# TruongKhang/cds-mvsnet

Hardware: AMD Instinct MI355X
Metric: depth-maps/sec per ref view at 640x512 N=5 D=192 (single-stage plane sweep incl. CostRegNet + regression) (higher is better)
Workload: dtype f32; 1 GPU; M1: single-stage StageNet volume 640x512, D=192, C=8, N=5 views; parallelism=single

## Files before the change

cds_mvsnet_amd/_lib.py:

```python
from __future__ import annotations

import ctypes
import os
from ctypes import c_float, c_int, c_longlong, c_void_p

_HERE = os.path.dirname(os.path.abspath(__file__))
LIB_PATH = os.environ.get("CDS_MVSNET_LIB") or os.path.join(_HERE, "libcdsmvs_hip.so")

ACT_NONE, ACT_RELU, ACT_LEAKY01, ACT_SIGMOID, ACT_TANH = 0, 1, 2, 3, 4
ACT_ACCUM = 16
AGG_ACCUMULATE, AGG_NORMALIZE, AGG_CHANNELS_LAST, AGG_FAST_POSITIONS = 1, 2, 4, 8
WARP_FAST_POSITIONS = AGG_FAST_POSITIONS
MAX_VIEWS = 8
MAX_IMAGES = 16
STAGE_STATE_WORDS = 2080
EINVAL = -1000

P = c_void_p
I = c_int
F = c_float
DB = ctypes.c_double
L = c_longlong

SIGNATURES = {
    "cds_version": [],
    "cds_chw_to_hwc_f32": [P, P, I, I, I, P],
    "cds_stage_inputs_f32": [P, P, P, P, P, P, P, P, P, P, I, I, I, I, P],
    "cds_homo_warp_f32": [P, P, P, P, I, I, I, I, I, P],
    "cds_warp_entropy_f32": [P, P, P, P, P, I, I, I, I, I, I, P],
    "cds_warp_entropy_flags_f32": [P, P, P, P, P, I, I, I, I, I, I, I, P],
    "cds_warp_aggregate_f32": [P, P, P, P, P, P, P, I, I, I, I, I, I, I, P],
    "cds_warp_entropy_window_f32": [P, P, P, P, P, I, I, I, I, I, I, I, I, P],
    "cds_warp_aggregate_window_f32": [P, P, P, P, P, P, P, I, I, I, I, I, I, I, I, P],
    "cds_warp_aggregate_bwd_f32": [P, P, P, P, P, P, P, P, P, I, I, I, I, I, I, P],
    "cds_volume_finish_f32": [P, P, P, I, I, I, I, P, P, P],
    "cds_volume_finish_bwd_f32": [P, P, P, P, P, I, I, I, I, P, P, P, P, P],
    "cds_volume_normalize_f32": [P, P, I, I, I, P],
    "cds_volume_normalize_cl_f32": [P, P, I, I, I, P],
    "cds_softargmin_conf_f32": [P, P, P, P, P, I, I, I, I, P],
    "cds_depth_hypotheses_f32": [P, P, I, I, I, I, I, I, P, P, P],
    "cds_depth_planes_f32": [P, I, I, I, P, P],
    "cds_conv3d_k3_f32": [P, P, P, P, P, I, I, I, I, I, I, I, P],
    "cds_conv3d_k3_cl_f32": [P, P, P, P, P, I, I, I, I, I, I, P],
    "cds_conv3d_sbf_f32": [P, P, P, P, P, I, I, I, I, I, I, I, P],
    "cds_conv3d_sf16_f32": [P, P, P, P, I, I, I, I, I, I, I, P, F, P, P],
    "cds_deconv3d_sbf_f32": [P, P, P, P, P, I, I, I, I, I, I, I, P],
    "cds_deconv3d_sf16_f32": [P, P, P, P, P, I, I, I, I, I, I, P, F, P, P],
    "cds_deconv3d_zm_sf16_f32": [P, P, P, P, P, I, I, I, I, I, I, P, F, P, P],
    "cds_deconv_prob_zm_f32": [P, P, P, P, P, P, I, I, I, P],
    "cds_deconv_prob_zm_sf16_f32": [P, P, P, P, P, P, I, I, I, P, F, P],
    "cds_deconv3d_zm_f32": [P, P, P, P, P, I, I, I, I, I, I, P],
    "cds_deconv3d_k3s2_f32": [P, P, P, P, P, I, I, I, I, I, I, P],
    "cds_conv2d_f32": [P, P, P, P, I, I, I, I, I, I, I, I, I, P],
    "cds_conv2d_affine_f32": [P, P, P, P, P, I, I, I, I, I, I, I, I, I, P],
    "cds_instnorm_affine_f32": [P, P, P, I, I, I, I, F, P],
    "cds_fpn_stats_parts": [I, I],
    "cds_conv2d_fpn_f32": [P, P, P, P, P, P, P, I, I, I, I, I, I, P],
    "cds_conv2d_k3_c16_f32": [P, P, P, P, P, P, I, I, I, I, P],
    "cds_dynconv_branches_sbf_f32": [P, P, P, P, P, I, I, I, I, I, P, I, P],
    "cds_dynconv_fused_sbf_f32": [P, P, P, P, P, P, P, P, F, P, P, P, I, I, I, I, I, P, I, P],
    "cds_dynconv_fused_parts": [I, I],
    "cds_conv2d_k3_relu_sbf_f32": [P, P, P, P, P, P, I, I, I, I, P],
    "cds_dynconv_blend_f32": [P, P, P, P, P, F, P, P, I, I, I, I, I, P],
    "cds_dynconv_blend_shared_f32": [P, P, P, P, P, F, P, P, I, I, I, I, I, I, P],
    "cds_blend_stats_parts": [I, I],
    "cds_dynconv_blend_stats_f32": [P, P, P, P, P, F, P, P, P, I, I, I, I, I, I, P],
    "cds_instnorm_reduce_f32": [P, I, P, P, I, I, I, I, F, P],
    "cds_instnorm_apply_f32": [P, P, P, I, I, I, I, I, I, P],
    "cds_instnorm_act_f32": [P, P, P, I, I, I, I, I, I, P],
    "cds_debug_poison_lds": [ctypes.c_uint],
    "cds_dynconv_cl_parts": [I, I],
    "cds_dynconv_cl_f32": [P, P, P, P, P, P, P, P, F, P, P, P, I, I, I, I, P, I, P],
    "cds_dynconv_cl_sf16_f32": [P, P, P, P, P, P, P, P, F, P, P, P, I, I, I, I, P, I, F, F, P],
    "cds_conv00_cl_f32": [P, P, P, P, P, P, P, F, P, P, P, I, I, I, I, P],
    "cds_conv00_cl_sf16_f32": [P, P, P, P, P, P, P, F, P, P, P, I, I, I, I, P, F, P],
    "cds_blend_cl_parts": [I, I],
    "cds_dynconv_blend_cl_f32": [P, P, P, P, P, F, P, P, P, I, I, I, I, I, I, P],
    "cds_conv2d_k3s2_cl_f32": [P, P, P, P, I, I, I, I, I, P],
    "cds_conv2d_k3s2_cl_sf16_f32": [P, P, P, P, I, I, I, I, I, F, F, P],
    "cds_fpn_cl_parts": [I, I],
    "cds_conv2d_fpn_cl_f32": [P, P, P, P, P, P, P, I, I, I, I, I, I, P],
    "cds_vis_layer1_cl_f32": [P, P, P, P, P, I, I, I, P],
    "cds_conv2d_k3_relu_cl_f32": [P, P, P, P, P, P, I, I, I, I, P],
    "cds_instnorm_stats_cl_parts": [I, I],
    "cds_instnorm_stats_cl_f32": [P, P, I, I, I, I, P],
    "cds_instnorm_apply_cl_f32": [P, P, P, P, I, I, I, I, I, I, I, P],
    "cds_curvature_stats_f32": [P, P, P, P, P, I, P],
    "cds_curvature_stats_bwd_f32": [P, P, P, P, P, P, P, P, I, P],
    "cds_pair_mean_f32": [P, P, I, I, P],
    "cds_view_mean_f32": [P, P, I, I, P],
    "cds_depth_affine_f32": [P, P, I, P, P],
    "cds_deconv2d_k3s2_f32": [P, P, P, P, I, I, I, I, I, P],
    "cds_refine_finish_f32": [P, P, P, I, I, P, P],
    "cds_bn3d_stats_f32": [P, P, I, I, L, P],
    "cds_bn3d_norm_f32": [P, P, P, P, DB, DB, F, P, P, P, P, P, P, P, P, I, I, L, I, P],
    "cds_bn3d_bwd_reduce_f32": [P, P, P, P, P, I, I, L, I, P],
    "cds_bn3d_bwd_norm_f32": [P, P, P, P, P, P, P, DB, P, P, P, I, I, L, I, P],
    "cds_conv3d_wgrad_f32": [P, P, P, I, I, I, I, I, I, I, I, I, I, P],
    "cds_bn3d_norm_bound_f32": [P, P, P, P, DB, DB, F, P, P, P, P, P, P, P, P, I, I, L, I, P, P],
    "cds_bn3d_bwd_norm_bound_f32": [P, P, P, P, P, P, P, DB, P, P, P, I, I, L, I, P, P],
    "cds_absmax_bound_f32": [P, L, P, P],
    "cds_sf16_pack_conv3d_f32": [P, P, P, P, I, I, I, P],
    "cds_conv3d_k3_sf16_f32": [P, P, P, P, P, I, I, I, I, I, I, I, P],
    "cds_conv3d_wgrad_sf16_f32": [P, P, P, P, P, I, I, I, I, I, I, I, I, I, I, P],
    "cds_conv2d_wgrad_f32": [P, P, P, I, I, I, I, I, I, I, I, I, I, P],
    "cds_conv2d_dgrad_s2_f32": [P, P, P, I, I, I, I, I, I, I, P],
    "cds_instnorm_bwd_f32": [P, P, P, P, P, I, I, I, I, I, I, P],
    "cds_dynconv_bn_stats_f32": [P, P, P, P, P, P, P, P, I, I, I, I, I, I, F, F, I, I, P],
    "cds_dynconv_blend_train_f32": [P, P, P, P, P, P, P, P, F, P, P, I, I, I, I, I, I, P],
    "cds_dynconv_blend_bwd_f32": [P, P, P, P, P, P, P, P, F, P, P, P, P, P, I, I, I, I, I, I, I, I, P],
    "cds_f32_to_bf16": [P, P, L, P],
    "cds_instnorm_act_b16_f32": [P, P, P, P, P, I, I, I, I, I, I, P],
    "cds_conv2d_wgrad_xb16_f32": [P, P, P, I, I, I, I, I, I, I, I, I, I, P],
    "cds_instnorm_bwd_yb16_f32": [P, P, P, P, P, P, I, I, I, I, I, I, P],
    "cds_dynconv_bn_stats_b16_f32": [P, P, P, P, P, P, P, P, I, I, I, I, I, I, F, F, I, I, P],
    "cds_dynconv_blend_train_b16_f32": [P, P, P, P, P, P, P, P, F, P, P, I, I, I, I, I, I, P],
    "cds_dynconv_blend_bwd_b16_f32": [P, P, P, P, P, P, P, P, F, P, P, P, P, P, I, I, I, I, I, I, I, I, P],
    "cds_pack_conv2d_f32": [P, P, P, P, I, I, I, I, P],
    "cds_pack_conv3d_f32": [P, P, P, I, I, I, P],
    "cds_softargmin_bwd_f32": [P, P, P, P, I, I, I, I, P],
    "cds_dynconv_bwd_finish_f32": [P, P, I, I, P, P],
    "cds_bn_running_update_f32": [P, P, P, F, I, I, P, P, P],
    "cds_loss_records": [ctypes.c_longlong],
    "cds_loss_stage_f32": [P, P, P, P, P, P, P, I, I, I, P, P, P],
    "cds_loss_final_f32": [P, P, P, P, P, P, I, P, P, P, P],
    "cds_loss_stage_bwd_f32": [P, P, P, P, P, P, P, P, F, I, I, I, P, P, P, P],
    "cds_feat_target_f32": [P, P, P, F, F, I, I, I, P, P],
    "cds_depth_fusion_f32": [P, P, P, P, P, P, P, P, P, I, I, I, P, F, F, F, P],
    "cds_grid_hash_log2_slots": [L],
    "cds_grid_keys_f32": [P, L, P, P, P],
    "cds_grid_hash_build": [P, L, L, P, P, I, P],
    "cds_nn_query_f32": [P, P, L, P, P, P, P, P, P, I, P, F, P, P],
    "cds_thin_round_f32": [P, P, L, P, P, I, P, F, P, P, P],
    "cds_gipuma_tiles": [L],
    "cds_gipuma_prob_filter_f32": [P, P, P, I, I, I, P, P, P, P],
    "cds_gipuma_fuse_view_f32": [P, P, P, P, I, I, I, I, F, F, F, I, P, P, P, P],
    "cds_gipuma_scan": [P, I, P, P, P, P],
    "cds_gipuma_compact_f32": [P, P, P, I, I, P, P, P, P],
    "cds_colmap_score_quantum_log2": [],
    "cds_colmap_score_limbs": [DB, DB, DB],
    "cds_colmap_pair_scores_f64": [P, P, P, P, P, P, L, L, I, DB, DB, DB, I, P, P],
    "cds_colmap_obs_depth_f64": [P, P, P, P, L, P, P],
    "cds_colmap_depth_ranges_f64": [P, P, P, P, I, P, P],
}

_lib = None


class CdsLibraryError(RuntimeError):
    pass


def load() -> ctypes.CDLL:
    global _lib
    if _lib is not None:
        return _lib
    if not os.path.exists(LIB_PATH):
        raise CdsLibraryError(
            f"{LIB_PATH} not found: build it with `make -C {os.path.join(_HERE, 'csrc')}` "
            "(or `python -c 'import __graft_entry__ as g; g.build()'`). "
            "cds_mvsnet_amd has no CPU / PyTorch fallback.")
    import torch

    lib = ctypes.CDLL(LIB_PATH)
    for name, argtypes in SIGNATURES.items():
        try:
            fn = getattr(lib, name)
        except AttributeError as e:
            raise CdsLibraryError(f"{LIB_PATH} does not export {name}") from e
        fn.argtypes = argtypes
        fn.restype = c_int
    _lib = lib
    return lib


def check(rc: int, what: str) -> None:
    if rc == 0:
        return
    if rc == EINVAL:
        raise ValueError(f"{what}: invalid argument (CDS_EINVAL)")
    raise RuntimeError(f"{what}: HIP error {-rc}")
```

cds_mvsnet_amd/csrc/cds_common.hpp:

```cpp
#pragma once
#include <hip/hip_runtime.h>
#include <stdint.h>
#include <stdlib.h>

#include <atomic>

#include "../../include/cds_mvsnet_hip.h"

#define CDS_WAVE 64

#define CDS_ZMG_UNSUPPORTED 1
int cds_conv3d_zmg_dispatch(const float* x, const void* wsp, const float* bias, float* out, int Cin, int Cout, int D, int H, int W,
                            int stride, int pair, int act, hipStream_t st, const float* in_bound = nullptr, float w_inv = 1.f,
                            float* out_bound = nullptr);

using cds_f4 = float __attribute__((ext_vector_type(4)));

extern "C" int cds_debug_poison_lds(unsigned pattern);

static inline int cds_launch_status() {
  hipError_t e = hipGetLastError();
  if (const char* p = getenv("CDS_DEBUG_POISON_LDS")) {
    if (e == hipSuccess) (void)cds_debug_poison_lds((unsigned)strtoul(p, nullptr, 16));
  }
  return e == hipSuccess ? 0 : -(int)e;
}

static inline int cds_ceil_div(int a, int b) { return (a + b - 1) / b; }

static inline bool cds_env_is(const char* name, char c) { const char* e = getenv(name); return e && e[0] == c; }
static inline bool cds_env_set(const char* name) { return getenv(name) != nullptr; }
static inline int cds_env_int(const char* name, int dflt) { const char* e = getenv(name); return e ? atoi(e) : dflt; }

static inline int cds_allow_lds(const void* kernel, int bytes, std::atomic<unsigned long long>& mask) {
  int d = 0;
  (void)hipGetDevice(&d);
  const unsigned long long bit = 1ull << (d & 63);
  if (mask.load(std::memory_order_acquire) & bit) return 0;
  hipError_t e = hipFuncSetAttribute(kernel, hipFuncAttributeMaxDynamicSharedMemorySize, bytes);
  if (e != hipSuccess) { (void)hipGetLastError(); return -(int)e; }
  mask.fetch_or(bit, std::memory_order_release);
  return 0;
}

__device__ __forceinline__ int cds_xcd_remap(int bid, int nwg) {
  const int nx = 8;
  if (nwg < 2 * nx) return bid;
  int q = nwg / nx, r = nwg % nx;
  int xcd = bid % nx, idx = bid / nx;
  int base = xcd < r ? xcd * (q + 1) : r * (q + 1) + (xcd - r) * q;
  return base + idx;
}

__device__ __forceinline__ const float* cds_uniform_ptr(const float* p) {
  const uint64_t u = reinterpret_cast<uint64_t>(p);
  const uint32_t lo = __builtin_amdgcn_readfirstlane((uint32_t)u);
  const uint32_t hi = __builtin_amdgcn_readfirstlane((uint32_t)(u >> 32));
  return reinterpret_cast<const float*>(((uint64_t)hi << 32) | lo);
}

__device__ __forceinline__ float cds_act_conv(float v, int act) {
  if (act == CDS_ACT_RELU) return fmaxf(v, 0.0f);
  if (act == CDS_ACT_SIGMOID) return 1.0f / (1.0f + expf(-v));
  return v;
}

__device__ __forceinline__ float cds_apply_act(float v, int act) {
  switch (act) {
    case CDS_ACT_RELU: return fmaxf(v, 0.0f);
    case CDS_ACT_LEAKY01: return v > 0.0f ? v : v * 0.1f;
    case CDS_ACT_SIGMOID: return 1.0f / (1.0f + expf(-v));
    case CDS_ACT_TANH: return tanhf(v);
    default: return v;
  }
}
```

cds_mvsnet_amd/csrc/conv3d_sbf.hip:

```cpp
#include <stdlib.h>

#include "cds_common.hpp"
#include "sbf_common.hpp"

namespace {

#ifdef CDS_SBF_XFAST
#define SBF_TILE(tile, A, B, C) const int A = (tile) % tiles_x, B = ((tile) / tiles_x) % tiles_y, C = (tile) / (tiles_x * tiles_y)
#else
#define SBF_TILE(tile, A, B, C) \
  const int tiles_z_ = ntiles / (tiles_x * tiles_y); \
  const int C = (tile) % tiles_z_, A = ((tile) / tiles_z_) % tiles_x, B = (tile) / (tiles_z_ * tiles_x)
#endif

template <int S, int MB, int TX_, int TZ_, bool PAIR = false, bool WRES_ = false>
struct FCfg {
  static constexpr int TX = TX_, TY = 4, TZ = TZ_;
  static constexpr bool DEINT = S == 2 || PAIR;
  static constexpr int XT = TX / (PAIR ? 32 : 16), NT = XT * TZ;
  static constexpr int IX = (TX - 1) * S + 3, IY = (TY - 1) * S + 3, IZ = (TZ - 1) * S + 3;
  static constexpr int IXH = DEINT ? (IX + 1) / 2 : 0;
  static constexpr int IXP = DEINT ? 2 * IXH : (IX + 7) / 8 * 8;
  static constexpr int NPOS = IZ * IY * IXP;
  static constexpr int LDSB = NPOS * POSB;
// ... 543 lines not shown
  }
  if (F16) sf16_publish_bound(amax, out_bound);
}

template <bool MERGE, int MB, bool F16 = false>
int launch_deconv(const float* x, const void* wsp, const float* b, const float* skip, float* out, int Cin, int Cout, int D, int H,
                  int W, int act, int out_planar, hipStream_t st, const float* in_bound = nullptr, float w_inv = 1.f,
                  float* out_bound = nullptr, int ysplit = 1) {
  using Cfg = DCfg;
  const int tx = cds_ceil_div(W, Cfg::CX), ty = cds_ceil_div(H, Cfg::CY);
  const int ntiles = tx * ty * D;
  int tpw = max(1, min(16, ntiles / (256 * 2 * 8)));
  const int nwg = cds_ceil_div(ntiles, tpw);
  hipLaunchKernelGGL((deconv3d_sbf_kernel<MERGE, MB, F16>), dim3(nwg, ysplit), dim3(256), Cfg::LDSB, st, x, reinterpret_cast<const uint4*>(wsp),
                     b, skip, out, Cin, Cout, D, H, W, act, out_planar, tx, ty, ntiles, tpw, in_bound, w_inv, out_bound);
  return cds_launch_status();
}

template <int CYT>
struct DWSCfg {
  static constexpr int CX = 32, CY = CYT;
  static constexpr int XT = CX / 16, NT = XT;
  static constexpr int IX = CX + 1, IY = CY + 1, IZ = 2;
  static constexpr int IXP = 40;
  static constexpr int NPOS = IZ * IY * IXP;
  static constexpr int LDSB = NPOS * POSB;
  static constexpr int CW = CYT, PW = CYT / 2, THREADS = (CW + PW) * 64;
};

#ifndef CDS_DWS_MINW
#define CDS_DWS_MINW 3
#endif
template <int CYT>
__global__ __launch_bounds__((DWSCfg<CYT>::THREADS), CDS_DWS_MINW) void deconv3d_sbf_ws_kernel(const float* __restrict__ x, const uint4* __restrict__ wsp,
                                                                       const float* __restrict__ bias, const float* __restrict__ skip,
                                                                       float* __restrict__ out, int Cin, int Cout, int D, int H, int W,
                                                                       int act, int out_planar, int tiles_x, int tiles_y, int ntiles,
                                                                       int tpw) {
  using Cfg = DWSCfg<CYT>;
  constexpr int DWS_CW = Cfg::CW, DWS_PW = Cfg::PW, DWS_THREADS = Cfg::THREADS;
  using Tab = DTab<true>;
  extern __shared__ __attribute__((aligned(16))) unsigned char lds[];
  const int tid = threadIdx.x;
  const int lane = tid & 63;
  const int wave = __builtin_amdgcn_readfirstlane(tid >> 6);
  const int nwg = gridDim.x;
  const int wg = cds_xcd_remap(blockIdx.x, nwg);
  const int tile0 = wg * tpw, tile1 = min(ntiles, tile0 + tpw);
  const int rounds = Cin >> 3;
  const int nstages = (tile1 - tile0) * rounds;
  if (nstages <= 0) return;
  const int wbytes = rounds * Tab::NKS * 3 * 1024;
  unsigned char* tiles = lds + wbytes;
  {
    uint4* wdst = reinterpret_cast<uint4*>(lds);
    for (int i = tid; i < wbytes / 16; i += DWS_THREADS) wdst[i] = wsp[i];
  }

  if (wave >= DWS_CW) {
    const int ptid = tid - DWS_CW * 64;
    constexpr int NP = Cfg::IZ * Cfg::IY * Cfg::IX;
    constexpr int PPT = (NP + DWS_PW * 64 - 1) / (DWS_PW * 64);
    int s_rel[PPT], s_dst[PPT];
#pragma unroll
    for (int h = 0; h < PPT; ++h) {
      const int p = h * DWS_PW * 64 + ptid;
      const int row = p / Cfg::IX, c = p - row * Cfg::IX;
      const int rz = row / Cfg::IY, ry = row - rz * Cfg::IY;
      s_rel[h] = p < NP ? ((rz << 20) | (ry << 10) | c) : -1;
      s_dst[h] = (row * Cfg::IXP + c) * POSB;
    }
    float4 va[2][PPT], vb[2][PPT];
    auto issue = [&](int st, int set) {
      const int tile = tile0 + st / rounds, rd = st % rounds;
      SBF_TILE(tile, tx_i, ty_i, az);
      const int gx0 = tx_i * Cfg::CX, gy0 = ty_i * Cfg::CY;
#pragma unroll
      for (int h = 0; h < PPT; ++h) {
        const int gz = az + (s_rel[h] >> 20), gy = gy0 + ((s_rel[h] >> 10) & 1023), gx = gx0 + (s_rel[h] & 1023);
        const bool ok = s_rel[h] >= 0 && gz < D && gy < H && gx < W;
        const float* __restrict__ src = x + ((size_t)((size_t)gz * H + gy) * W + gx) * Cin + rd * 8;
        va[set][h] = ok ? *reinterpret_cast<const float4*>(src) : make_float4(0.f, 0.f, 0.f, 0.f);
        vb[set][h] = ok ? *reinterpret_cast<const float4*>(src + 4) : make_float4(0.f, 0.f, 0.f, 0.f);
      }
    };
    auto deposit = [&](int buf, int set) {
      unsigned char* base = tiles + buf * Cfg::LDSB;
#pragma unroll
      for (int h = 0; h < PPT; ++h)
        if (s_rel[h] >= 0) split_store8(base + s_dst[h], va[set][h], vb[set][h]);
    };
    issue(0, 0);
    if (nstages > 1) issue(1, 1);
    deposit(0, 0);
    if (nstages > 2) issue(2, 0);
    __syncthreads();
    for (int st = 0; st < nstages; st += 2) {
      if (st + 1 < nstages) {
        deposit(1, 1);
        if (st + 3 < nstages) issue(st + 3, 1);
      }
      __syncthreads();
      if (st + 1 >= nstages) break;
      if (st + 2 < nstages) {
        deposit(0, 0);
        if (st + 4 < nstages) issue(st + 4, 0);
      }
      __syncthreads();
    }
    return;
  }

  SBF_CONSUMER_PRIO();
  const int j = lane & 15, g = lane >> 4;
  int toff[Tab::NKS];
#pragma unroll
  for (int ks = 0; ks < Tab::NKS; ++ks) {
    const int c = Tab::cls_of(ks), s0 = Tab::slot0_of(ks);
    int off = 0;
#pragma unroll
    for (int gg = 0; gg < 4; ++gg) {
      const int dz = Tab::tap_d(c, s0 + gg, 0), dy = Tab::tap_d(c, s0 + gg, 1), dx = Tab::tap_d(c, s0 + gg, 2);
      const int o = dz < 0 ? 0 : ((dz * Cfg::IY + dy) * Cfg::IXP + dx) * POSB;
      off = g == gg ? o : off;
    }
    toff[ks] = off;
  }
  const int b_base = (wave * Cfg::IXP + j) * POSB;
  const unsigned char* wlds = lds + lane * 16;
  const int co = 4 * (g & 1), px = g >> 1;
  const float4 bv = bias ? *reinterpret_cast<const float4*>(bias + co) : make_float4(0.f, 0.f, 0.f, 0.f);
  const int Ho = 2 * H, Wo = 2 * W;
  f32x4 acc[Tab::NCLS][Cfg::NT];
  float4 skv[Tab::NCLS][Cfg::NT];
  __syncthreads();
  int st = 0;
  for (int tile = tile0; tile < tile1; ++tile) {
    SBF_TILE(tile, tx_i, ty_i, az);
    const int ay = ty_i * Cfg::CY + wave;
#pragma unroll
    for (int c = 0; c < Tab::NCLS; ++c)
#pragma unroll
      for (int t = 0; t < Cfg::NT; ++t) acc[c][t] = (f32x4){0.f, 0.f, 0.f, 0.f};
    if (skip && ay < H) {
#pragma unroll
      for (int c = 0; c < Tab::NCLS; ++c) {
        const size_t rowbase = ((size_t)(2 * az + (c >> 1)) * Ho + (2 * ay + (c & 1))) * Wo;
#pragma unroll
        for (int q = 0; q < Cfg::NT; ++q) {
          const int ax = min(tx_i * Cfg::CX + q * 16 + j, W - 1);
          skv[c][q] = *reinterpret_cast<const float4*>(skip + (rowbase + 2 * ax + px) * Cout + co);
        }
      }
    }
    for (int rd = 0; rd < rounds; ++rd, ++st) {
      const unsigned char* tbuf = tiles + (st & 1) * Cfg::LDSB;
      const unsigned char* wr = wlds + rd * Tab::NKS * 3 * 1024;
      BV wa[2][3];
      BV bd[2][Cfg::NT][3];
      auto load_w = [&](int buf, int ks) {
        wa[buf][0].u = *reinterpret_cast<const uint4*>(wr + (ks * 3) * 1024);
        wa[buf][1].u = *reinterpret_cast<const uint4*>(wr + (ks * 3 + 1) * 1024);
        wa[buf][2].u = *reinterpret_cast<const uint4*>(wr + (ks * 3 + 2) * 1024);
      };
      auto load_b = [&](int buf, int ks) {
        const unsigned char* bp = tbuf + b_base + toff[ks];
#pragma unroll
        for (int q = 0; q < Cfg::NT; ++q) {
          const unsigned char* b = bp + q * 16 * POSB;
          bd[buf][q][0].u = *reinterpret_cast<const uint4*>(b);
          bd[buf][q][1].u = *reinterpret_cast<const uint4*>(b + 16);
          bd[buf][q][2].u = *reinterpret_cast<const uint4*>(b + 32);
        }
      };
      load_w(0, 0);
      load_b(0, 0);
#pragma unroll
      for (int ks = 0; ks < Tab::NKS; ++ks) {
        const int c = Tab::cls_of(ks), cur = ks & 1;
        if (ks + 1 < Tab::NKS) {
          load_b(cur ^ 1, ks + 1);
          load_w(cur ^ 1, ks + 1);
        }
        __builtin_amdgcn_sched_barrier(0);
        SBF_TERMS(acc[c], 0, Cfg::NT, wa[cur], bd[cur]);
      }
      if (rd + 1 == rounds && ay < H) {
#pragma unroll
        for (int c = 0; c < Tab::NCLS; ++c) {
          const size_t rowbase = ((size_t)(2 * az + (c >> 1)) * Ho + (2 * ay + (c & 1))) * Wo;
#pragma unroll
          for (int q = 0; q < Cfg::NT; ++q) {
            const int ax = tx_i * Cfg::CX + q * 16 + j;
            if (ax >= W) continue;
            const size_t base = (rowbase + 2 * ax + px) * Cout + co;
            const f32x4 a = acc[c][q];
            float4 o = make_float4(a.x + bv.x, a.y + bv.y, a.z + bv.z, a.w + bv.w);
            if (act == CDS_ACT_RELU) {
              o.x = fmaxf(o.x, 0.f); o.y = fmaxf(o.y, 0.f); o.z = fmaxf(o.z, 0.f); o.w = fmaxf(o.w, 0.f);
            }
            if (skip) {
              const float4 s4 = skv[c][q];
              o.x = s4.x + o.x; o.y = s4.y + o.y; o.z = s4.z + o.z; o.w = s4.w + o.w;
            }
            if (out_planar) {
              const size_t ovol = (size_t)(2 * D) * Ho * Wo;
              float* po = out + (size_t)co * ovol + (rowbase + 2 * ax + px);
#ifdef CDS_SBF_NTSTORE
              __builtin_nontemporal_store(o.x, po); __builtin_nontemporal_store(o.y, po + ovol);
              __builtin_nontemporal_store(o.z, po + 2 * ovol); __builtin_nontemporal_store(o.w, po + 3 * ovol);
#else
              po[0] = o.x; po[ovol] = o.y; po[2 * ovol] = o.z; po[3 * ovol] = o.w;
#endif
            } else {
              sbf_store4(out + base, o);
            }
          }
        }
      }
      __syncthreads();
    }
  }
}

template <int CYT>
int launch_deconv_ws_t(const float* x, const void* wsp, const float* b, const float* skip, float* out, int Cin, int Cout, int D, int H,
                       int W, int act, int out_planar, hipStream_t st) {
  using Cfg = DWSCfg<CYT>;
  const int tx = cds_ceil_div(W, Cfg::CX), ty = cds_ceil_div(H, Cfg::CY);
  const int ntiles = tx * ty * D;
  int tpw = max(1, min(16, ntiles / (256 * (CYT == 8 ? 1 : 2) * 8)));
  const int nwg = cds_ceil_div(ntiles, tpw);
  const int lds_bytes = (Cin >> 3) * DTab<true>::NKS * 3 * 1024 + 2 * Cfg::LDSB;
  static std::atomic<unsigned long long> lds_ok{0};
  if (int e_lds = cds_allow_lds(reinterpret_cast<const void*>(deconv3d_sbf_ws_kernel<CYT>), 160 * 1024, lds_ok)) return e_lds;
  hipLaunchKernelGGL(deconv3d_sbf_ws_kernel<CYT>, dim3(nwg), dim3(Cfg::THREADS), lds_bytes, st, x, reinterpret_cast<const uint4*>(wsp), b,
                     skip, out, Cin, Cout, D, H, W, act, out_planar, tx, ty, ntiles, tpw);
  return cds_launch_status();
}

int launch_deconv_ws(const float* x, const void* wsp, const float* b, const float* skip, float* out, int Cin, int Cout, int D, int H,
                     int W, int act, int out_planar, hipStream_t st) {
  const bool big = (H >= 16 && (long)cds_ceil_div(W, 32) * cds_ceil_div(H, 8) * D >= 2 * 256);
  if (big) return launch_deconv_ws_t<8>(x, wsp, b, skip, out, Cin, Cout, D, H, W, act, out_planar, st);
  return launch_deconv_ws_t<4>(x, wsp, b, skip, out, Cin, Cout, D, H, W, act, out_planar, st);
}

}

extern "C" int cds_conv3d_sbf_f32(const float* x, const void* weight_split, const float* bias, const float* skip, float* out,
                                  int Cin, int Cout, int D, int H, int W, int stride, int act, void* stream) {
  if (!x || !weight_split || !out || Cin < 8 || (Cin % 8) || Cout < 4 || (Cout % 4) || Cout > 64 || D < 1 || H < 1 || W < 1 ||
      (stride != 1 && stride != 2 && stride != CDS_SBF_PAIR))
    return CDS_EINVAL;
  if (stride == CDS_SBF_PAIR && Cout != 8) return CDS_EINVAL;
  hipStream_t st = (hipStream_t)stream;
  const int mb = (Cout + 15) / 16;
  if (!skip) {
    const int r = cds_conv3d_zmg_dispatch(x, weight_split, bias, out, Cin, Cout, D, H, W, stride == CDS_SBF_PAIR ? 1 : stride,
                                          stride == CDS_SBF_PAIR, act, st);
    if (r != CDS_ZMG_UNSUPPORTED) return r;
  }
  if (stride == CDS_SBF_PAIR) {
    if (Cout != 8) return CDS_EINVAL;
    if (Cin == 8) return launch_fwd<1, 1, 32, 4, true, true>(x, weight_split, bias, skip, out, Cin, Cout, D, H, W, act, st);
    return launch_fwd<1, 1, 32, 4, true>(x, weight_split, bias, skip, out, Cin, Cout, D, H, W, act, st);
  }
  if (stride == 1) {
    if (mb == 1) return launch_fwd<1, 1, 32, 4>(x, weight_split, bias, skip, out, Cin, Cout, D, H, W, act, st);
    if (mb == 2) return launch_fwd<1, 2, 32, 2>(x, weight_split, bias, skip, out, Cin, Cout, D, H, W, act, st);
    if (mb == 4) return launch_fwd<1, 4, 32, 2>(x, weight_split, bias, skip, out, Cin, Cout, D, H, W, act, st);
    return CDS_EINVAL;
  }
  if (mb == 1) return launch_fwd<2, 1, 16, 2>(x, weight_split, bias, skip, out, Cin, Cout, D, H, W, act, st);
  if (mb == 2) return launch_fwd<2, 2, 16, 2>(x, weight_split, bias, skip, out, Cin, Cout, D, H, W, act, st);
  if (mb == 4) return launch_fwd<2, 4, 16, 2>(x, weight_split, bias, skip, out, Cin, Cout, D, H, W, act, st);
  return CDS_EINVAL;
}

extern "C" int cds_conv3d_sf16_f32(const float* x, const void* weight_split, const float* bias, float* out, int Cin, int Cout, int D, int H,
                                   int W, int stride, int act, const float* in_bound, float w_inv_scale, float* out_bound, void* stream) {
  if (!x || !weight_split || !out || !in_bound || Cin < 8 || (Cin % 8) || Cout < 4 || (Cout % 4) || Cout > 64 || D < 1 || H < 1 || W < 1 ||
      (stride != 1 && stride != 2 && stride != CDS_SBF_PAIR) || !(w_inv_scale > 0.f))
    return CDS_EINVAL;
  if (stride == CDS_SBF_PAIR && Cout != 8) return CDS_EINVAL;
  hipStream_t st = (hipStream_t)stream;
  const int r = cds_conv3d_zmg_dispatch(x, weight_split, bias, out, Cin, Cout, D, H, W, stride == CDS_SBF_PAIR ? 1 : stride,
                                        stride == CDS_SBF_PAIR, act, st, in_bound, w_inv_scale, out_bound);
  if (r != CDS_ZMG_UNSUPPORTED) return r;
  const int mb = (Cout + 15) / 16;
  const int s_ = stride, Do = (D - 1) / s_ + 1, Ho = (H - 1) / s_ + 1, Wo = (W - 1) / s_ + 1;
  const long tiles = (long)cds_ceil_div(Wo, s_ == 1 ? 32 : 16) * cds_ceil_div(Ho, 4) * cds_ceil_div(Do, 2);
  const bool split = tiles <= cds_env_int("CDS_SBF_YSPLIT_TILES", 256) && !cds_env_is("CDS_SBF_YSPLIT", '0');
  if (split && stride == 1 && (mb == 2 || mb == 4))
    return launch_fwd<1, 1, 32, 2, false, false, true>(x, weight_split, bias, nullptr, out, Cin, Cout, D, H, W, act, st, in_bound, w_inv_scale, out_bound, mb);
  if (split && stride == 2 && mb == 4)
    return launch_fwd<2, 1, 16, 2, false, false, true>(x, weight_split, bias, nullptr, out, Cin, Cout, D, H, W, act, st, in_bound, w_inv_scale, out_bound, mb);
  if (stride == 1 && mb == 2) return launch_fwd<1, 2, 32, 2, false, false, true>(x, weight_split, bias, nullptr, out, Cin, Cout, D, H, W, act, st, in_bound, w_inv_scale, out_bound);
  if (stride == 1 && mb == 4) return launch_fwd<1, 4, 32, 2, false, false, true>(x, weight_split, bias, nullptr, out, Cin, Cout, D, H, W, act, st, in_bound, w_inv_scale, out_bound);
  if (stride == 2 && mb == 4) return launch_fwd<2, 4, 16, 2, false, false, true>(x, weight_split, bias, nullptr, out, Cin, Cout, D, H, W, act, st, in_bound, w_inv_scale, out_bound);
  return CDS_EINVAL;
}

extern "C" int cds_deconv3d_sf16_f32(const float* x, const void* weight_split, const float* bias, const float* skip, float* out, int Cin,
                                     int Cout, int D, int H, int W, int act, const float* in_bound, float w_inv_scale, float* out_bound,
                                     void* stream) {
  if (!x || !weight_split || !out || !in_bound || Cin < 8 || (Cin % 8) || Cout != 32 || D < 1 || H < 1 || W < 1 || !(w_inv_scale > 0.f))
    return CDS_EINVAL;
  const long tiles = (long)cds_ceil_div(W, 32) * cds_ceil_div(H, 4) * D;
  if (tiles <= cds_env_int("CDS_SBF_YSPLIT_TILES", 256) && !cds_env_is("CDS_SBF_YSPLIT", '0'))
    return launch_deconv<false, 1, true>(x, weight_split, bias, skip, out, Cin, Cout, D, H, W, act, 0, (hipStream_t)stream, in_bound,
                                         w_inv_scale, out_bound, 2);
  return launch_deconv<false, 2, true>(x, weight_split, bias, skip, out, Cin, Cout, D, H, W, act, 0, (hipStream_t)stream, in_bound,
                                       w_inv_scale, out_bound);
}

extern "C" int cds_deconv3d_sbf_f32(const float* x, const void* weight_split, const float* bias, const float* skip, float* out,
                                    int Cin, int Cout, int D, int H, int W, int act, int out_planar, void* stream) {
  if (!x || !weight_split || !out || Cin < 8 || (Cin % 8) || D < 1 || H < 1 || W < 1) return CDS_EINVAL;
  hipStream_t st = (hipStream_t)stream;
  if (Cout == 8) {
    if (Cin <= 32) return launch_deconv_ws(x, weight_split, bias, skip, out, Cin, Cout, D, H, W, act, out_planar, st);
    return launch_deconv<true, 1>(x, weight_split, bias, skip, out, Cin, Cout, D, H, W, act, out_planar, st);
  }
  if (Cout == 16) return launch_deconv<false, 1>(x, weight_split, bias, skip, out, Cin, Cout, D, H, W, act, out_planar, st);
  if (Cout == 32) return launch_deconv<false, 2>(x, weight_split, bias, skip, out, Cin, Cout, D, H, W, act, out_planar, st);
  return CDS_EINVAL;
}
```

cds_mvsnet_amd/csrc/conv3d_zmg.hip:

```cpp
#include <stdlib.h>

#include "cds_common.hpp"
#include "sbf_common.hpp"

namespace {

__device__ __attribute__((aligned(32))) float g_zmg_zeros[8];

template <int S_, int RD_, int MB_, bool PAIR_, int TXO_, int TYO_, int G_, int NG_, int CW_ = 4, bool F16_ = false, int RPW_ = 1,
          int YS_ = 1, int PF_ = 1>
struct ZG {
  static constexpr int S = S_, RD = RD_, MB = MB_, TXO = TXO_, TYO = TYO_, G = G_, NG = NG_;
  static constexpr bool F16 = F16_;
  static constexpr int NT = F16_ ? 2 : 3;
  static constexpr bool PAIR = PAIR_, DEINT = PAIR_ || S_ == 2;
  static constexpr int CW = CW_, PW = 4, THREADS = (CW + PW) * 64;
  static constexpr int RPW = RPW_, YS = YS_, PF = PF_;
  static_assert(PF == 1 || (PF == 2 && 2 * NG_ * (F16_ ? 2 : 3) <= 15), "operand prefetch distance (lgkmcnt is a 4-bit count)");
  static_assert(RD % RPW == 0 && MB % YS == 0, "rounds per wave / cout split");
  static constexpr int KSPL = RD / RPW, MBS = MB / YS;
  static_assert(CW % (KSPL * MBS) == 0 && (KSPL == 1 || KSPL == 2 || KSPL == 4), "consumer waves");
  static constexpr int PARTS = CW / (KSPL * MBS);
  static constexpr int ROWS = TYO / PARTS;
  static constexpr int XT = TXO / (PAIR ? 32 : 16);
  static constexpr int NTW = ROWS * XT * G;
  static_assert(TYO % PARTS == 0 && NTW % NG == 0 && (KSPL != 2 || NTW % 2 == 0), "tile split");
  static constexpr int KW = PAIR ? 4 : 3, KS = (9 * KW + 3) / 4;
  static constexpr int IX = (TXO - 1) * S + 3, IY = (TYO - 1) * S + 3;
  static constexpr int IXH = DEINT ? (IX + 1) / 2 : 0;
  static constexpr int IXP = DEINT ? 2 * IXH : IX;
  static constexpr int SLICEB = IY * IXP * POSB, PLANEB = RD * SLICEB;
  static constexpr int NINIT = 3 - S;
  static constexpr int NRES = S * (G - 1) + 3, NNEW = S * G, R = NRES + NNEW;
  static constexpr int RINGB = R * PLANEB;
  static constexpr int XCH1 = KSPL == 2 ? CW * (NTW / 2) * 1024 : (KSPL == 4 ? CW * NTW * 1024 : 0);
  static constexpr int NFIN = KSPL == 4 ? (NTW + 3) / 4 : 1;
  static constexpr int tap_of(int t, int gg) {
    const int tap = PAIR ? 4 * t + ((gg & 1) * 2 + (gg >> 1)) : 4 * t + gg;
    return tap > 9 * KW - 1 ? 9 * KW - 1 : tap;
  }
  static constexpr int tap_kz(int t, int gg) { return tap_of(t, gg) / (3 * KW); }
  static constexpr int tap_off(int t, int gg) {
    const int tap = tap_of(t, gg), ky = (tap / KW) % 3, kx = tap % KW;
    return (ky * IXP + (DEINT ? ((kx & 1) * IXH + (kx >> 1)) : kx)) * POSB;
  }
  static constexpr int LDSB = RINGB + 2 * XCH1;
  static_assert(LDSB <= 160 * 1024, "LDS budget");
  static constexpr int NITEM = NNEW * IY * RD * IXP;
  static constexpr int PT = PW * 64, PPT = (NITEM + PT - 1) / PT;
};

template <class Cfg>
__global__ __launch_bounds__(Cfg::THREADS, 1) void conv3d_zmg_kernel(const float* __restrict__ x, const uint4* __restrict__ wsp,
                                                                  const float* __restrict__ bias, float* __restrict__ out, int Cout,
                                                                  int D, int H, int W, int Do, int Ho, int Wo, int act,
                                                                  int tiles_x, int tiles_y, int zseg,
                                                                  const float* __restrict__ in_bound, float w_inv,
                                                                  float* __restrict__ out_bound) {
  constexpr int S = Cfg::S, RD = Cfg::RD, G = Cfg::G, R = Cfg::R, Cin = 8 * RD, KS = Cfg::KS, NTW = Cfg::NTW, NG = Cfg::NG;
  constexpr bool PAIR = Cfg::PAIR, F16 = Cfg::F16;
  constexpr int NT = Cfg::NT;
  const float xs = F16 ? sf16_scale(in_bound[0]) : 1.0f;
  const float out_mul = F16 ? w_inv / xs : 1.0f;
  extern __shared__ __attribute__((aligned(16))) unsigned char lds[];
  const int tid = threadIdx.x;
  const int lane = tid & 63;
  const int wave = __builtin_amdgcn_readfirstlane(tid >> 6);
  const int nseg = (Do + zseg - 1) / zseg;
  int unit = cds_xcd_remap(blockIdx.x, gridDim.x);
  const int seg = unit % nseg;
  unit /= nseg;
  const int tx_i = unit % tiles_x, ty_i = unit / tiles_x;
  const int z0 = seg * zseg, z1 = min(Do, z0 + zseg);
  const int nstages = (z1 - z0 + G - 1) / G;
  const int gx0 = tx_i * Cfg::TXO * S - 1, gy0 = ty_i * Cfg::TYO * S - 1;
  const int zin0 = S * z0 - 1;

  if (wave >= Cfg::CW) {
#ifndef CDS_ZMG_PPRIO
#define CDS_ZMG_PPRIO 3
#endif
    __builtin_amdgcn_s_setprio(CDS_ZMG_PPRIO);
    constexpr int PT = Cfg::PT, PPT = Cfg::PPT;
    const int ptid = tid - Cfg::CW * 64;
    int s_pl[PPT], s_dst[PPT];
    long long s_off[PPT];
    unsigned okmask = 0;
#pragma unroll
    for (int h = 0; h < PPT; ++h) {
      const int p = h * PT + ptid;
      const int q = p % Cfg::IXP, t1 = p / Cfg::IXP;
      const int rd = t1 % RD, t2 = t1 / RD;
      const int row = t2 % Cfg::IY, pl = t2 / Cfg::IY;
      const int c = Cfg::DEINT ? (2 * (q % Cfg::IXH) + q / Cfg::IXH) : q;
      const int gy = gy0 + row, gx = gx0 + c;
      const bool exists = p < Cfg::NITEM && c < Cfg::IX;
      s_pl[h] = pl;
      s_dst[h] = rd * Cfg::SLICEB + (row * Cfg::IXP + q) * POSB;
      s_off[h] = ((long long)gy * W + gx) * Cin + rd * 8;
      if (exists && (unsigned)gy < (unsigned)H && (unsigned)gx < (unsigned)W) okmask |= 1u << h;
      if (!exists) s_pl[h] = -1;
    }
    const long long plane_elems = (long long)H * W * Cin;
    float4 va[2][PPT], vb[2][PPT];
    auto issue = [&](int st, int set) {
      const int zn = zin0 + st * S * G + Cfg::NINIT;
#pragma unroll
      for (int h = 0; h < PPT; ++h) {
        const int z = zn + s_pl[h];
        const bool ok = ((okmask >> h) & 1u) && (unsigned)z < (unsigned)D;
        const float* __restrict__ src = ok ? x + ((long long)z * plane_elems + s_off[h]) : g_zmg_zeros;
        va[set][h] = *reinterpret_cast<const float4*>(src);
        vb[set][h] = *reinterpret_cast<const float4*>(src + 4);
      }
    };
    auto deposit = [&](int st, int set) {
      const int slot0 = (st * S * G + Cfg::NINIT) % R;
#pragma unroll
      for (int h = 0; h < PPT; ++h) {
        if (h + 1 == PPT && s_pl[h] < 0) continue;
        int slot = slot0 + (s_pl[h] < 0 ? 0 : s_pl[h]);
        slot = slot >= R ? slot - R : slot;
        if (F16) split_store8_f16(lds + slot * Cfg::PLANEB + s_dst[h], va[set][h], vb[set][h], xs);
        else split_store8(lds + slot * Cfg::PLANEB + s_dst[h], va[set][h], vb[set][h]);
      }
    };
    for (int p = ptid; p < Cfg::NINIT * Cfg::IY * RD * Cfg::IXP; p += PT) {
      const int q = p % Cfg::IXP, t1 = p / Cfg::IXP;
      const int rd = t1 % RD, t2 = t1 / RD;
      const int row = t2 % Cfg::IY, pl = t2 / Cfg::IY;
      const int c = Cfg::DEINT ? (2 * (q % Cfg::IXH) + q / Cfg::IXH) : q;
      const int gz = zin0 + pl, gy = gy0 + row, gx = gx0 + c;
      const bool ok = c < Cfg::IX && (unsigned)gz < (unsigned)D && (unsigned)gy < (unsigned)H && (unsigned)gx < (unsigned)W;
      const float* __restrict__ src = ok ? x + (((long long)gz * H + gy) * W + gx) * Cin + rd * 8 : g_zmg_zeros;
      if (F16)
        split_store8_f16(lds + pl * Cfg::PLANEB + rd * Cfg::SLICEB + (row * Cfg::IXP + q) * POSB, *reinterpret_cast<const float4*>(src),
                         *reinterpret_cast<const float4*>(src + 4), xs);
      else
        split_store8(lds + pl * Cfg::PLANEB + rd * Cfg::SLICEB + (row * Cfg::IXP + q) * POSB, *reinterpret_cast<const float4*>(src),
                     *reinterpret_cast<const float4*>(src + 4));
    }
    issue(0, 0);
    if (nstages > 1) issue(1, 1);
    deposit(0, 0);
    if (nstages > 2) issue(2, 0);
    __syncthreads();
    for (int st = 0; st < nstages; st += 2) {
      if (st + 1 < nstages) {
        deposit(st + 1, 1);
        if (st + 3 < nstages) issue(st + 3, 1);
      }
      __syncthreads();
      if (st + 1 >= nstages) break;
      if (st + 2 < nstages) {
        deposit(st + 2, 0);
        if (st + 4 < nstages) issue(st + 4, 0);
      }
      __syncthreads();
    }
    return;
  }

#ifndef CDS_ZMG_CPRIO
#define CDS_ZMG_CPRIO 2
#endif
  __builtin_amdgcn_s_setprio(CDS_ZMG_CPRIO);
  const int k = wave % Cfg::KSPL, mbi = (wave / Cfg::KSPL) % Cfg::MBS, part = wave / (Cfg::KSPL * Cfg::MBS);
  const int j = lane & 15, g = lane >> 4;
#ifdef CDS_ZMG_NOSKEW
  const bool late = false;
#else
  const bool late = Cfg::CW == 8 && wave >= 4;
#endif
  const int lane_base = k * Cfg::RPW * Cfg::SLICEB + (part * Cfg::ROWS * S * Cfg::IXP + j) * POSB +
                        (PAIR ? (((g & 1) * 2 + (g >> 1)) & 1) * Cfg::IXH * POSB + ((((g & 1) * 2 + (g >> 1))) >> 1) * POSB : 0);
  constexpr int RPW = Cfg::RPW;
  const int mbg = (Cfg::YS > 1 ? blockIdx.y * Cfg::MBS : 0) + mbi;
  BV wres[RPW * KS][NT];
  {
    const uint4* __restrict__ wl = wsp + lane;
#pragma unroll
    for (int t = 0; t < RPW * KS; ++t) {
      const size_t o = (size_t)(((k * RPW * KS + t) * Cfg::MB + mbg) * 3) * 64;
#pragma unroll
      for (int tm = 0; tm < NT; ++tm) wres[t][tm].u = wl[o + 64 * tm];
    }
  }
  float amax = 0.f;
  const int co = PAIR ? 4 * (g & 1) : mbg * 16 + 4 * g;
  const float4 bv = (bias && co < Cout) ? *reinterpret_cast<const float4*>(bias + co) : make_float4(0.f, 0.f, 0.f, 0.f);
  constexpr int XW = PAIR ? 32 : 16;
  const int oy0 = ty_i * Cfg::TYO + part * Cfg::ROWS;
  const int ox0 = tx_i * Cfg::TXO + (PAIR ? 2 * j + (g >> 1) : j);
  float* const obase = out + ((size_t)((size_t)z0 * Ho + oy0) * Wo + ox0) * Cout + co;
  bool lane_ok[Cfg::XT];
#pragma unroll
  for (int xt = 0; xt < Cfg::XT; ++xt) lane_ok[xt] = ox0 + xt * XW < Wo && co < Cout;
  auto store_tile = [&](int n, int st, const f32x4& a) {
    const int i = n % G, rx = n / G, xt = rx % Cfg::XT, r = rx / Cfg::XT;
    if (z0 + st * G + i >= z1 || oy0 + r >= Ho) return;
    if (!lane_ok[xt]) return;
    float4 o = F16 ? make_float4(a.x * out_mul + bv.x, a.y * out_mul + bv.y, a.z * out_mul + bv.z, a.w * out_mul + bv.w)
                   : make_float4(a.x + bv.x, a.y + bv.y, a.z + bv.z, a.w + bv.w);
    if (act == CDS_ACT_RELU) {
      o.x = fmaxf(o.x, 0.f); o.y = fmaxf(o.y, 0.f); o.z = fmaxf(o.z, 0.f); o.w = fmaxf(o.w, 0.f);
    }
    if (F16) amax = fmaxf(fmaxf(amax, fmaxf(fabsf(o.x), fabsf(o.y))), fmaxf(fabsf(o.z), fabsf(o.w)));
    sbf_store4(obase + ((size_t)((size_t)(st * G + i) * Ho + r) * Wo + xt * XW) * Cout, o);
  };
  unsigned char* xch = lds + Cfg::RINGB;
  constexpr int NH = NTW / 2;
  f32x4 acc[NTW];
  constexpr bool KEEP4 = Cfg::RPW == 1;
  f32x4 keep[Cfg::KSPL == 2 ? NH : Cfg::NFIN];
  auto store_tile_rt = [&](int n, int st, const f32x4& a) {
    const int i = n % G, rx = n / G, xt = rx % Cfg::XT, r = rx / Cfg::XT;
    if (z0 + st * G + i >= z1 || oy0 + r >= Ho) return;
    if (!(ox0 + xt * XW < Wo && co < Cout)) return;
    float4 o = F16 ? make_float4(a.x * out_mul + bv.x, a.y * out_mul + bv.y, a.z * out_mul + bv.z, a.w * out_mul + bv.w)
                   : make_float4(a.x + bv.x, a.y + bv.y, a.z + bv.z, a.w + bv.w);
    if (act == CDS_ACT_RELU) {
      o.x = fmaxf(o.x, 0.f); o.y = fmaxf(o.y, 0.f); o.z = fmaxf(o.z, 0.f); o.w = fmaxf(o.w, 0.f);
    }
    if (F16) amax = fmaxf(fmaxf(amax, fmaxf(fabsf(o.x), fabsf(o.y))), fmaxf(fabsf(o.z), fabsf(o.w)));
    sbf_store4(obase + ((size_t)((size_t)(st * G + i) * Ho + r) * Wo + xt * XW) * Cout, o);
  };
  const int xgrp = (wave / Cfg::KSPL) * NTW;
  auto finish = [&](int sp) {
    if (Cfg::KSPL == 2) {
      const unsigned char* src = xch + (sp & 1) * Cfg::XCH1 + ((wave ^ 1) * NH) * 1024 + lane * 16;
#pragma unroll
      for (int m = 0; m < NH; ++m) {
        const f32x4 o = *reinterpret_cast<const f32x4*>(src + m * 1024);
        store_tile(k * NH + m, sp, k == 0 ? keep[m] + o : o + keep[m]);
      }
    } else if (Cfg::KSPL == 4) {
#pragma unroll
      for (int jf = 0; jf < Cfg::NFIN; ++jf) {
        const int n = jf * 4 + k;
        if (n >= NTW) continue;
        const unsigned char* src = xch + (sp & 1) * Cfg::XCH1 + ((xgrp + n) * 4) * 1024 + lane * 16;
        f32x4 total = KEEP4 && k == 0 ? keep[jf] : *reinterpret_cast<const f32x4*>(src);
#pragma unroll
        for (int kk = 1; kk < 4; ++kk) total = total + (KEEP4 && kk == k ? keep[jf] : *reinterpret_cast<const f32x4*>(src + kk * 1024));
        store_tile_rt(n, sp, total);
      }
    } else {
#pragma unroll
      for (int n = 0; n < NTW; ++n) store_tile(n, sp, acc[n]);
    }
  };
  __syncthreads();
  for (int st = 0; st < nstages; ++st) {
    if (late && st > 0) finish(st - 1);
    int vpl[PAIR ? Cfg::NRES : 1];
    int vaddr[PAIR ? 1 : KS][PAIR ? 1 : G];
    {
      int sl[Cfg::NRES];
      int slot = (st * S * G) % R;
#pragma unroll
      for (int u = 0; u < Cfg::NRES; ++u) {
        sl[u] = slot * Cfg::PLANEB;
        slot = slot + 1 >= R ? slot + 1 - R : slot + 1;
      }
      if (PAIR) {
#pragma unroll
        for (int u = 0; u < Cfg::NRES; ++u) vpl[u] = lane_base + sl[u];
      } else {
#pragma unroll
        for (int t = 0; t < KS; ++t)
#pragma unroll
          for (int i = 0; i < G; ++i) {
            const int o0 = sl[S * i + Cfg::tap_kz(t, 0)] + Cfg::tap_off(t, 0), o1 = sl[S * i + Cfg::tap_kz(t, 1)] + Cfg::tap_off(t, 1);
            const int o2 = sl[S * i + Cfg::tap_kz(t, 2)] + Cfg::tap_off(t, 2), o3 = sl[S * i + Cfg::tap_kz(t, 3)] + Cfg::tap_off(t, 3);
            vaddr[t][i] = lane_base + (g == 0 ? o0 : (g == 1 ? o1 : (g == 2 ? o2 : o3)));
          }
      }
    }
    constexpr int NGRP = NTW / NG, NS = RPW * KS * NGRP;
    constexpr int PF = Cfg::PF;
    BV bd[PF + 1][NG][NT];
    auto load_b = [&](int buf, int ss) {
      const int t = (ss / NGRP) % KS, rr = ss / (NGRP * KS), grp = ss % NGRP;
#pragma unroll
      for (int q = 0; q < NG; ++q) {
        const int n = grp * NG + q, i = n % G, rx = n / G, xt = rx % Cfg::XT, r = rx / Cfg::XT;
        const unsigned char* b = lds + (PAIR ? vpl[PAIR ? S * i + t / 3 : 0] + (t % 3) * Cfg::IXP * POSB : vaddr[PAIR ? 0 : t][PAIR ? 0 : i]) +
                                 (r * S * Cfg::IXP + xt * 16) * POSB + rr * Cfg::SLICEB;
        bd[buf][q][0].u = *reinterpret_cast<const uint4*>(b);
        bd[buf][q][1].u = *reinterpret_cast<const uint4*>(b + 16);
        if (!F16) bd[buf][q][NT - 1].u = *reinterpret_cast<const uint4*>(b + 32);
      }
    };
    load_b(0, 0);
    if (PF == 2 && NS > 1) load_b(1, 1);
    __builtin_amdgcn_s_setprio(0);
#pragma unroll
    for (int t = 0; t < NTW; ++t) acc[t] = (f32x4){0.f, 0.f, 0.f, 0.f};
#pragma unroll
    for (int ss = 0; ss < NS; ++ss) {
      const int t = ss / NGRP, grp = ss % NGRP, db = ss % (PF + 1);
      if (ss + PF < NS) load_b((ss + PF) % (PF + 1), ss + PF);
      __builtin_amdgcn_sched_barrier(0);
#ifndef CDS_ZMG_LAZYWAIT
      if (ss + PF < NS) __builtin_amdgcn_s_waitcnt(0xC07F | ((PF * NT * NG) << 8));
      else if (PF == 2 && ss + 1 < NS) __builtin_amdgcn_s_waitcnt(0xC07F | ((NT * NG) << 8));
      else __builtin_amdgcn_s_waitcnt(0xC07F);
      __builtin_amdgcn_sched_barrier(0);
#endif
      if constexpr (F16) {
        SF16_TERMS(acc, grp * NG, NG, wres[t], bd[db]);
      } else {
        SBF_TERMS(acc, grp * NG, NG, wres[t], bd[db]);
      }
    }
    __builtin_amdgcn_s_setprio(CDS_ZMG_CPRIO);
    if (Cfg::KSPL == 2) {
      if (!late && st > 0) finish(st - 1);
      unsigned char* dst = xch + (st & 1) * Cfg::XCH1 + (wave * NH) * 1024 + lane * 16;
#pragma unroll
      for (int m = 0; m < NH; ++m) {
        *reinterpret_cast<f32x4*>(dst + m * 1024) = acc[(k ^ 1) * NH + m];
        keep[m] = acc[k * NH + m];
      }
    } else if (Cfg::KSPL == 4) {
      if (!late && st > 0) finish(st - 1);
      unsigned char* dst = xch + (st & 1) * Cfg::XCH1 + (xgrp * 4 + k) * 1024 + lane * 16;
#pragma unroll
      for (int n = 0; n < NTW; ++n) {
        if (KEEP4 && (n & 3) == k) keep[n >> 2] = acc[n];
        else *reinterpret_cast<f32x4*>(dst + n * 4096) = acc[n];
      }
    } else if (!late) {
      finish(st);
    }
    __syncthreads();
  }
  if (Cfg::KSPL >= 2 || late) finish(nstages - 1);
  if (F16) sf16_publish_bound(amax, out_bound);
}

inline int zmg_pick_nseg(int cols, int Do, int G) {
  const int nseg_env = cds_env_int("CDS_ZMG_NSEG", 0);
  if (nseg_env > 0) return nseg_env;
  const int stages = cds_ceil_div(Do, G);
  int best = 1;
  double best_cost = 1e30;
  for (int n = 1; n <= 32 && n <= stages; ++n) {
    const int per = cds_ceil_div(stages, n);
    if (n > 1 && per < 6) break;
    const double cost = (double)cds_ceil_div(cols * cds_ceil_div(stages, per), 256) * (per + 2.5);
    if (cost < best_cost - 1e-9) { best_cost = cost; best = n; }
  }
  return best;
}

template <class Cfg>
int launch_zmg(const float* x, const void* wsp, const float* b, float* out, int Cout, int D, int H, int W, int act, hipStream_t st,
               const float* in_bound = nullptr, float w_inv = 1.f, float* out_bound = nullptr, int min_wgs = 0) {
  constexpr int S = Cfg::S;
  const int Do = (D - 1) / S + 1, Ho = (H - 1) / S + 1, Wo = (W - 1) / S + 1;
  const int tx = cds_ceil_div(Wo, Cfg::TXO), ty = cds_ceil_div(Ho, Cfg::TYO);
  int nseg = zmg_pick_nseg(tx * ty * Cfg::YS, Do, Cfg::G);
  const int zseg = cds_ceil_div(cds_ceil_div(Do, nseg), Cfg::G) * Cfg::G;
  nseg = cds_ceil_div(Do, zseg);
  if (min_wgs > 0 && tx * ty * nseg * Cfg::YS < min_wgs) return CDS_ZMG_UNSUPPORTED;
  auto kern = conv3d_zmg_kernel<Cfg>;
  static std::atomic<unsigned long long> lds_ok{0};
  if (int e_lds = cds_allow_lds(reinterpret_cast<const void*>(kern), Cfg::LDSB, lds_ok)) return e_lds;
  hipLaunchKernelGGL(kern, dim3(tx * ty * nseg, Cfg::YS), dim3(Cfg::THREADS), Cfg::LDSB, st, x, reinterpret_cast<const uint4*>(wsp), b,
                     out, Cout, D, H, W, Do, Ho, Wo, act, tx, ty, zseg, in_bound, w_inv, out_bound);
  return cds_launch_status();
}

}

int cds_conv3d_zmg_dispatch(const float* x, const void* wsp, const float* bias, float* out, int Cin, int Cout, int D, int H, int W,
                            int stride, int pair, int act, hipStream_t st, const float* in_bound, float w_inv, float* out_bound) {
  if (in_bound) {
    if (pair) {
      if (Cin == 8) return launch_zmg<ZG<1, 1, 1, true, 32, 8, 3, 1, 8, true>>(x, wsp, bias, out, Cout, D, H, W, act, st, in_bound, w_inv, out_bound);
      if (Cin == 16) return launch_zmg<ZG<1, 2, 1, true, 32, 8, 1, 4, 4, true>>(x, wsp, bias, out, Cout, D, H, W, act, st, in_bound, w_inv, out_bound);
      if (Cin == 32) return launch_zmg<ZG<1, 4, 1, true, 32, 3, 1, 3, 4, true>>(x, wsp, bias, out, Cout, D, H, W, act, st, in_bound, w_inv, out_bound);
      return CDS_ZMG_UNSUPPORTED;
    }
    if (stride == 1 && Cin == 16 && Cout == 16)
      return launch_zmg<ZG<1, 2, 1, false, 32, 8, 1, 1, 8, true>>(x, wsp, bias, out, Cout, D, H, W, act, st, in_bound, w_inv, out_bound);
    if (stride == 2 && Cin == 8 && Cout == 16)
      return launch_zmg<ZG<2, 1, 1, false, 16, 8, 1, 1, 8, true>>(x, wsp, bias, out, Cout, D, H, W, act, st, in_bound, w_inv, out_bound);
    if (stride == 2 && Cin == 16 && Cout == 32)
      return launch_zmg<ZG<2, 2, 2, false, 16, 4, 1, 1, 8, true>>(x, wsp, bias, out, Cout, D, H, W, act, st, in_bound, w_inv, out_bound);
    const int deep = cds_env_is("CDS_ZMG", '0') ? 0 : cds_env_int("CDS_ZMG_DEEP", 1);
    const int min_wgs = deep == 2 ? 0 : 256;
    if (deep > 0 && stride == 1 && Cin == 32 && Cout == 32)
      return launch_zmg<ZG<1, 4, 2, false, 16, 4, 1, 1, 8, true, 1, 1, 2>>(x, wsp, bias, out, Cout, D, H, W, act, st, in_bound, w_inv, out_bound, min_wgs);
    if (deep > 0 && stride == 1 && Cin == 64 && Cout == 64)
      return launch_zmg<ZG<1, 8, 4, false, 16, 2, 1, 1, 8, true, 2, 2>>(x, wsp, bias, out, Cout, D, H, W, act, st, in_bound, w_inv, out_bound, min_wgs);
    return CDS_ZMG_UNSUPPORTED;
  }
  const bool off = cds_env_is("CDS_ZMG", '0');
  if (off) return CDS_ZMG_UNSUPPORTED;
  if (pair) {
    if (Cin == 8) return launch_zmg<ZG<1, 1, 1, true, 32, 8, 3, 1, 8>>(x, wsp, bias, out, Cout, D, H, W, act, st);
    if (Cin == 16) return launch_zmg<ZG<1, 2, 1, true, 32, 8, 1, 4>>(x, wsp, bias, out, Cout, D, H, W, act, st);
    if (Cin == 32) return launch_zmg<ZG<1, 4, 1, true, 32, 3, 1, 3>>(x, wsp, bias, out, Cout, D, H, W, act, st);
    return CDS_ZMG_UNSUPPORTED;
  }
  if (stride == 1) {
    if (Cin == 16 && Cout == 16) return launch_zmg<ZG<1, 2, 1, false, 32, 8, 1, 1, 8>>(x, wsp, bias, out, Cout, D, H, W, act, st);
    return CDS_ZMG_UNSUPPORTED;
  }
  if (Cin == 8 && Cout == 16) return launch_zmg<ZG<2, 1, 1, false, 16, 8, 1, 1, 8>>(x, wsp, bias, out, Cout, D, H, W, act, st);
  if (Cin == 16 && Cout == 32) return launch_zmg<ZG<2, 2, 2, false, 16, 4, 1, 1, 8>>(x, wsp, bias, out, Cout, D, H, W, act, st);
  return CDS_ZMG_UNSUPPORTED;
}
```

cds_mvsnet_amd/ops.py:

```python
from __future__ import annotations

import ctypes
import os
from typing import Optional, Tuple

import torch

from . import _lib
from ._lib import (ACT_LEAKY01, ACT_NONE, ACT_RELU, ACT_SIGMOID, ACT_TANH, AGG_ACCUMULATE, AGG_CHANNELS_LAST, AGG_FAST_POSITIONS,
                   AGG_NORMALIZE,
                   MAX_IMAGES, MAX_VIEWS, check)

Tensor = torch.Tensor

PROFILE_ON = False
PROFILE: dict = {}
PROFILE_HOST_MS: dict = {}


class prof:

    def __init__(self, name: str):
        self.name = name
        self.start = None
# ... 326 lines not shown


def softargmin_conf(prob_pre: Tensor, hyp: Tensor, want_prob: bool = False):
    D, h, w = prob_pre.shape
    D2, pp = _hyp_args(hyp, D, h, w)
    if D2 != D:
        raise ValueError("softargmin_conf: hypotheses / volume depth mismatch")
    depth = torch.empty((h, w), dtype=torch.float32, device=prob_pre.device)
    conf = torch.empty_like(depth)
    prob = torch.empty_like(prob_pre) if want_prob else None
    with prof("softargmin_conf"):
        check(_lib.load().cds_softargmin_conf_f32(_dev(prob_pre, "prob_pre"), _dev(hyp, "hyp"), depth.data_ptr(),
                                                  conf.data_ptr(), prob.data_ptr() if want_prob else None, D, h, w, pp,
                                                  _stream(depth)), "cds_softargmin_conf_f32")
    return (depth, conf, prob) if want_prob else (depth, conf)


def depth_hypotheses(prev_depth: Tensor, D: int, H: int, W: int, scale: int, interval, dmin, dmax=None) -> Tensor:
    hp, wp = prev_depth.shape
    dev = prev_depth.device
    out = torch.empty((D, H // scale, W // scale), dtype=torch.float32, device=dev)
    if dmax is None:
        ival, rng = geo(interval, dev, "interval"), geo(dmin, dev, "depth_range")
    else:
        ival = geo([interval, dmin, dmax], dev, "interval")
        rng = ival[1:]
    if ival.numel() < 1 or rng.numel() < 2:
        raise ValueError("depth_hypotheses: interval needs 1 value, the depth range 2")
    check(_lib.load().cds_depth_hypotheses_f32(_dev(prev_depth, "prev_depth"), out.data_ptr(), D, hp, wp, H, W, scale,
                                               _dev(ival, "interval"), _dev(rng, "depth_range"), _stream(out)),
          "cds_depth_hypotheses_f32")
    return out


def depth_planes(D: int, h: int, w: int, lo, hi, device) -> Tensor:
    out = torch.empty((D, h, w), dtype=torch.float32, device=device)
    rng = geo(lo if hi is None else [lo, hi], out.device, "depth_range")
    if rng.numel() < 2:
        raise ValueError("depth_planes: the depth range needs 2 values")
    check(_lib.load().cds_depth_planes_f32(out.data_ptr(), D, h, w, _dev(rng, "depth_range"), _stream(out)),
          "cds_depth_planes_f32")
    return out


USE_CONV3D_CL = os.environ.get("CDS_CONV_CL", "1") != "0"


def conv3d_cl_supported(Cin: int, Cout: int, W: int, stride: int) -> bool:
    return stride == 1 and Cin % 16 == 0 and Cout % 16 == 0 and W % 4 == 0 and W >= 16 and USE_CONV3D_CL


def conv3d_cl_preferred(Cin: int) -> bool:
    return Cin >= 64 or os.environ.get("CDS_CONV_CL", "1") == "2"


def conv3d_k3(x: Tensor, wpk: Tensor, bias: Optional[Tensor], stride: int = 1, relu: bool = True,
              skip: Optional[Tensor] = None, wcl: Optional[Tensor] = None) -> Tensor:
    Cin, D, H, W = x.shape
    if (wcl is not None and conv3d_cl_supported(Cin, wpk.shape[2], W, stride) and conv3d_cl_preferred(Cin)
            and Cin * D * H * W < 0x7fffffff):
        Cout = wpk.shape[2]
        if tuple(wcl.shape) != (27, Cout, Cin):
            raise ValueError("conv3d_k3: wcl must be [27,Cout,Cin]")
        out = torch.empty((Cout, D, H, W), dtype=torch.float32, device=x.device)
        if skip is not None and skip.shape != out.shape:
            raise ValueError("conv3d_k3: residual shape mismatch")
        check(_lib.load().cds_conv3d_k3_cl_f32(_dev(x, "x"), _dev(wcl, "weight_cl"), _dev(bias, "bias") if bias is not None else None,
                                               _dev(skip, "skip") if skip is not None else None, out.data_ptr(), Cin, Cout,
                                               D, H, W, ACT_RELU if relu else ACT_NONE, _stream(x)), "cds_conv3d_k3_cl_f32")
        return out
    if wpk.shape[0] != Cin or wpk.shape[1] != 27:
        raise ValueError("conv3d_k3: packed weight must be [Cin,27,Cout]")
    Cout = wpk.shape[2]
    Do, Ho, Wo = (D - 1) // stride + 1, (H - 1) // stride + 1, (W - 1) // stride + 1
    out = torch.empty((Cout, Do, Ho, Wo), dtype=torch.float32, device=x.device)
    if skip is not None and skip.shape != out.shape:
        raise ValueError("conv3d_k3: residual shape mismatch")
    check(_lib.load().cds_conv3d_k3_f32(_dev(x, "x"), _dev(wpk, "weight"), _dev(bias, "bias") if bias is not None else None,
                                        _dev(skip, "skip") if skip is not None else None, out.data_ptr(), Cin, Cout, D, H,
                                        W, stride, ACT_RELU if relu else ACT_NONE, _stream(x)), "cds_conv3d_k3_f32")
    return out


def split_pack_conv3d(w: Tensor, f16: bool = False):
    Cout, Cin = w.shape[:2]
    if Cin % 8:
        raise ValueError("split_pack_conv3d: Cin must be a multiple of 8")
    rounds, mbl = Cin // 8, (Cout + 15) // 16
    taps = torch.zeros((mbl * 16, rounds, 28, 8), dtype=torch.float32, device=w.device)
    taps[:Cout, :, :27] = w.detach().float().reshape(Cout, rounds, 8, 27).permute(0, 1, 3, 2)
    a = taps.reshape(mbl, 16, rounds, 7, 4, 8).permute(2, 3, 0, 4, 1, 5).reshape(rounds, 7, mbl, 64, 8)
    return _split2_f16(a) if f16 else _split3(a)


def _split2_f16(a: Tensor) -> Tuple[Tensor, float]:
    import math
    m = float(a.abs().max())
    e = math.frexp(m)[1] if (m > 0.0 and math.isfinite(m)) else 15
    e = max(-100, min(100, e))
    s = 2.0 ** (15 - e)
    v = a * s
    hi = v.to(torch.float16)
    lo = (v - hi.float()).to(torch.float16)
    return torch.stack((hi, lo, torch.zeros_like(hi)), dim=-3).contiguous().view(torch.int16), 1.0 / s


def _split3(a: Tensor) -> Tensor:
    hi = a.to(torch.bfloat16)
    r1 = a - hi.float()
    mid = r1.to(torch.bfloat16)
    lo = (r1 - mid.float()).to(torch.bfloat16)
    return torch.stack((hi, mid, lo), dim=-3).contiguous().view(torch.int16)


def _deconv_tables(merge: bool):
    ax = {0: [(1, 0)], 1: [(2, 0), (0, 1)]}
    if merge:
        classes = [(pz, py, None) for pz in (0, 1) for py in (0, 1)]
        ksteps = [(0, 0), (1, 0), (2, 0), (3, 0), (3, 4)]
    else:
        classes = [(pz, py, px) for pz in (0, 1) for py in (0, 1) for px in (0, 1)]
        ksteps = [(c, 0) for c in range(8)] + [(7, 4)]
    taps = []
    for pz, py, px in classes:
        tl = []
        for kz, dz in ax[pz]:
            for ky, dy in ax[py]:
                for xs in ([0, 1] if merge else ax[px]):
                    tl.append((kz, ky, xs))
        taps.append(tl)
    return classes, ksteps, taps


def split_pack_deconv3d(w: Tensor, f16: bool = False):
    Cin, Cout = w.shape[:2]
    if Cin % 8 or Cout not in (8, 16, 32):
        raise ValueError("split_pack_deconv3d: Cin % 8 == 0 and Cout in {8, 16, 32}")
    merge = Cout == 8
    mbl = 1 if merge else Cout // 16
    rounds = Cin // 8
    _, ksteps, taps = _deconv_tables(merge)
    wf = w.detach().float().reshape(rounds, 8, Cout, 3, 3, 3)
    a = torch.zeros((rounds, len(ksteps), mbl, 4, 16, 8), dtype=torch.float32, device=w.device)
    for ks, (c, s0) in enumerate(ksteps):
        for gg in range(4):
            s = s0 + gg
            if s >= len(taps[c]):
                continue
            kz, ky, xs = taps[c][s]
            if merge:
                dx = xs
                if dx == 0:
                    a[:, ks, 0, gg, 0:8] = wf[:, :, :, kz, ky, 1].permute(0, 2, 1)
                    a[:, ks, 0, gg, 8:16] = wf[:, :, :, kz, ky, 2].permute(0, 2, 1)
                else:
                    a[:, ks, 0, gg, 8:16] = wf[:, :, :, kz, ky, 0].permute(0, 2, 1)
            else:
                kx = xs[0]
                for mb in range(mbl):
                    a[:, ks, mb, gg] = wf[:, :, mb * 16:(mb + 1) * 16, kz, ky, kx].permute(0, 2, 1)
    a = a.reshape(rounds, len(ksteps), mbl, 64, 8)
    return _split2_f16(a) if f16 else _split3(a)


def deconv3d_sbf(x_cl: Tensor, wsplit: Tensor, bias: Optional[Tensor], cout: int, relu: bool = True,
                 skip: Optional[Tensor] = None, out_planar: bool = False, in_bound: Optional[Tensor] = None, w_inv_scale: float = 1.0,
                 out_bound: Optional[Tensor] = None) -> Tensor:
    D, H, W, Cin = x_cl.shape
    out = torch.empty((cout, 2 * D, 2 * H, 2 * W) if out_planar else (2 * D, 2 * H, 2 * W, cout), dtype=torch.float32,
                      device=x_cl.device)
    if skip is not None and tuple(skip.shape) != (2 * D, 2 * H, 2 * W, cout):
        raise ValueError("deconv3d_sbf: residual shape mismatch")
    if wsplit.dtype != torch.int16 or not wsplit.is_cuda or not wsplit.is_contiguous():
        raise ValueError("deconv3d_sbf: wsplit must be the contiguous int16 device tensor from split_pack_deconv3d")
    if in_bound is not None:
        if cout != 32 or out_planar:
            raise ValueError("deconv3d_sbf: the split-f16 form exists for cout == 32, channels-last output")
        check(_lib.load().cds_deconv3d_sf16_f32(_dev(x_cl, "x"), wsplit.data_ptr(), _dev(bias, "bias") if bias is not None else None,
                                                _dev(skip, "skip") if skip is not None else None, out.data_ptr(), Cin, cout, D, H, W,
                                                ACT_RELU if relu else ACT_NONE, _dev(in_bound, "in_bound"), float(w_inv_scale),
                                                _dev(out_bound, "out_bound") if out_bound is not None else None, _stream(x_cl)),
              "cds_deconv3d_sf16_f32")
        return out
    check(_lib.load().cds_deconv3d_sbf_f32(_dev(x_cl, "x"), wsplit.data_ptr(), _dev(bias, "bias") if bias is not None else None,
                                           _dev(skip, "skip") if skip is not None else None, out.data_ptr(), Cin, cout,
                                           D, H, W, ACT_RELU if relu else ACT_NONE, 1 if out_planar else 0, _stream(x_cl)),
          "cds_deconv3d_sbf_f32")
    return out


def split_pack_deconv_cls(w: Tensor, f16: bool = False):
    if tuple(w.shape) != (32, 16, 3, 3, 3):
        raise ValueError("split_pack_deconv_cls: ConvTranspose3d weight [32,16,3,3,3]")
    wf = w.detach().float().reshape(4, 8, 16, 3, 3, 3)
    a = torch.zeros((8, 4, 2, 4, 16, 8), dtype=torch.float32, device=w.device)
    tap = lambda par, d: (1 if d == 0 else None) if par == 0 else (2 if d == 0 else 0)
    for c in range(8):
        pz, py, px = c >> 2, (c >> 1) & 1, c & 1
        for dz in range(2):
            for g in range(4):
                kz, ky, kx = tap(pz, dz), tap(py, g >> 1), tap(px, g & 1)
                if kz is None or ky is None or kx is None:
                    continue
                a[c, :, dz, g] = wf[:, :, :, kz, ky, kx].permute(0, 2, 1)
    a = a.reshape(8, 4, 2, 64, 8)
    return _split2_f16(a) if f16 else _split3(a)


def deconv3d_zm(x_cl: Tensor, wcls: Tensor, bias: Optional[Tensor], relu: bool = True, skip: Optional[Tensor] = None,
                in_bound: Optional[Tensor] = None, w_inv_scale: float = 1.0, out_bound: Optional[Tensor] = None) -> Tensor:
    D, H, W, Cin = x_cl.shape
    out = torch.empty((2 * D, 2 * H, 2 * W, 16), dtype=torch.float32, device=x_cl.device)
    if skip is not None and tuple(skip.shape) != tuple(out.shape):
        raise ValueError("deconv3d_zm: residual shape mismatch")
    if wcls.dtype != torch.int16 or not wcls.is_cuda or not wcls.is_contiguous() or wcls.numel() != 8 * 4 * 2 * 3 * 64 * 8:
        raise ValueError("deconv3d_zm: wcls must be the contiguous int16 device tensor from split_pack_deconv_cls")
    if in_bound is not None:
        check(_lib.load().cds_deconv3d_zm_sf16_f32(_dev(x_cl, "x"), wcls.data_ptr(), _dev(bias, "bias") if bias is not None else None,
                                                   _dev(skip, "skip") if skip is not None else None, out.data_ptr(), Cin, 16, D, H, W,
                                                   ACT_RELU if relu else ACT_NONE, _dev(in_bound, "in_bound"), float(w_inv_scale),
                                                   _dev(out_bound, "out_bound") if out_bound is not None else None, _stream(x_cl)),
              "cds_deconv3d_zm_sf16_f32")
        return out
    check(_lib.load().cds_deconv3d_zm_f32(_dev(x_cl, "x"), wcls.data_ptr(), _dev(bias, "bias") if bias is not None else None,
                                          _dev(skip, "skip") if skip is not None else None, out.data_ptr(), Cin, 16, D, H, W,
                                          ACT_RELU if relu else ACT_NONE, _stream(x_cl)), "cds_deconv3d_zm_f32")
    return out


def split_pack_deconv_prob(w: Tensor, f16: bool = False):
    if tuple(w.shape) != (16, 8, 3, 3, 3):
        raise ValueError("split_pack_deconv_prob: ConvTranspose3d weight [16,8,3,3,3]")
    wf = w.detach().float().reshape(2, 8, 8, 3, 3, 3)
    a = torch.zeros((2, 5, 4, 16, 8), dtype=torch.float32, device=w.device)
    ops_tab = [
        [(1, 1), None],
        [(1, 2), (1, 0)],
        [(2, 1), (0, 1)],
        [(2, 2), (0, 2)],
        [(2, 0), (0, 0)],
    ]
    for k, groups in enumerate(ops_tab):
        for hi, kk in enumerate(groups):
            if kk is None:
                continue
            kz, ky = kk
            a[:, k, 2 * hi, 0:8] = wf[:, :, :, kz, ky, 1].permute(0, 2, 1)
            a[:, k, 2 * hi, 8:16] = wf[:, :, :, kz, ky, 2].permute(0, 2, 1)
            a[:, k, 2 * hi + 1, 8:16] = wf[:, :, :, kz, ky, 0].permute(0, 2, 1)
    a = a.reshape(2, 5, 64, 8)
    return _split2_f16(a) if f16 else _split3(a)


def pack_prob_table(w: Tensor) -> Tensor:
    if tuple(w.shape) != (1, 8, 3, 3, 3):
        raise ValueError("pack_prob_table: Conv3d weight [1,8,3,3,3]")
    return w.detach().float()[0].reshape(2, 4, 3, 3, 3).permute(4, 0, 3, 2, 1).contiguous()


def deconv_prob_zm(x_cl: Tensor, wsplit: Tensor, bias: Tensor, skip: Tensor, prob_table: Tensor, in_bound: Optional[Tensor] = None,
                   w_inv_scale: float = 1.0) -> Tensor:
    D, H, W, Cin = x_cl.shape
    if Cin != 16 or tuple(skip.shape) != (2 * D, 2 * H, 2 * W, 8):
        raise ValueError("deconv_prob_zm: x [D,H,W,16] and skip [2D,2H,2W,8]")
    if wsplit.dtype != torch.int16 or not wsplit.is_cuda or not wsplit.is_contiguous() or wsplit.numel() != 2 * 5 * 3 * 64 * 8:
        raise ValueError("deconv_prob_zm: wsplit must be the contiguous int16 device tensor from split_pack_deconv_prob")
    if prob_table.numel() != 216 or bias.numel() != 8:
        raise ValueError("deconv_prob_zm: prob_table from pack_prob_table, bias [8]")
    out = torch.empty((2 * D, 2 * H, 2 * W), dtype=torch.float32, device=x_cl.device)
    if in_bound is not None:
        check(_lib.load().cds_deconv_prob_zm_sf16_f32(_dev(x_cl, "x"), wsplit.data_ptr(), _dev(bias, "bias"), _dev(skip, "skip"),
                                                      _dev(prob_table, "prob_table"), out.data_ptr(), D, H, W, _dev(in_bound, "in_bound"),
                                                      float(w_inv_scale), _stream(x_cl)), "cds_deconv_prob_zm_sf16_f32")
        return out
    check(_lib.load().cds_deconv_prob_zm_f32(_dev(x_cl, "x"), wsplit.data_ptr(), _dev(bias, "bias"), _dev(skip, "skip"),
                                             _dev(prob_table, "prob_table"), out.data_ptr(), D, H, W, _stream(x_cl)),
          "cds_deconv_prob_zm_f32")
    return out


SBF_PAIR = 101
USE_SPLIT_F16 = os.environ.get("CDS_SPLIT_F16", "1") != "0"


def split_pack_conv3d_pair(w: Tensor, f16: bool = False):
    Cout, Cin = w.shape[:2]
    if Cout != 8 or Cin % 8:
        raise ValueError("split_pack_conv3d_pair: Cout == 8 and Cin % 8 == 0")
    rounds = Cin // 8
    wf = w.detach().float().reshape(8, rounds, 8, 3, 3, 3)
    taps = torch.zeros((2, 8, rounds, 3, 3, 4, 8), dtype=torch.float32, device=w.device)
    for p_ in (0, 1):
        taps[p_, :, :, :, :, p_:p_ + 3] = wf.permute(0, 1, 3, 4, 5, 2)
    taps = taps[:, :, :, :, :, [0, 2, 1, 3]]
    a = taps.reshape(16, rounds, 9, 4, 8).permute(1, 2, 3, 0, 4).reshape(rounds, 9, 1, 64, 8)
    return _split2_f16(a) if f16 else _split3(a)


def conv3d_sf16_supported(cin: int, cout: int, stride: int) -> bool:
    return USE_SPLIT_F16 and (cin, cout, stride) in ((8, 8, SBF_PAIR), (16, 8, SBF_PAIR), (32, 8, SBF_PAIR), (16, 16, 1), (8, 16, 2), (16, 32, 2),
                                                     (32, 32, 1), (32, 64, 2), (64, 64, 1))


def conv3d_sbf(x_cl: Tensor, wsplit: Tensor, bias: Optional[Tensor], cout: int, stride: int = 1, relu: bool = True,
               skip: Optional[Tensor] = None, in_bound: Optional[Tensor] = None, w_inv_scale: float = 1.0,
               out_bound: Optional[Tensor] = None) -> Tensor:
    D, H, W, Cin = x_cl.shape
    sg = 1 if stride == SBF_PAIR else stride
    Do, Ho, Wo = (D - 1) // sg + 1, (H - 1) // sg + 1, (W - 1) // sg + 1
    out = torch.empty((Do, Ho, Wo, cout), dtype=torch.float32, device=x_cl.device)
    if skip is not None and skip.shape != out.shape:
        raise ValueError("conv3d_sbf: residual shape mismatch")
    if wsplit.dtype != torch.int16 or not wsplit.is_cuda or not wsplit.is_contiguous():
        raise ValueError("conv3d_sbf: wsplit must be the contiguous int16 device tensor from split_pack_conv3d")
    if stride == SBF_PAIR and cout != 8:
        raise ValueError("conv3d_sbf: the pair-packed form (stride=SBF_PAIR) exists for cout == 8 only")
    ksteps = 9 if stride == SBF_PAIR else 7
    want = (Cin // 8) * ksteps * ((cout + 15) // 16) * 3 * 64 * 8
    if Cin % 8 or wsplit.numel() != want:
        raise ValueError(f"conv3d_sbf: wsplit has {wsplit.numel()} entries, the packer gives {want} for Cin={Cin}, cout={cout}, "
                         f"stride code {stride}")
    if in_bound is not None:
        if skip is not None or not conv3d_sf16_supported(Cin, cout, stride):
            raise ValueError(f"conv3d_sbf: no split-f16 kernel for Cin={Cin}, cout={cout}, stride code {stride}, skip={skip is not None}")
        check(_lib.load().cds_conv3d_sf16_f32(_dev(x_cl, "x"), wsplit.data_ptr(), _dev(bias, "bias") if bias is not None else None,
                                              out.data_ptr(), Cin, cout, D, H, W, stride, ACT_RELU if relu else ACT_NONE,
                                              _dev(in_bound, "in_bound"), float(w_inv_scale),
                                              _dev(out_bound, "out_bound") if out_bound is not None else None, _stream(x_cl)),
              "cds_conv3d_sf16_f32")
        return out
    check(_lib.load().cds_conv3d_sbf_f32(_dev(x_cl, "x"), wsplit.data_ptr(), _dev(bias, "bias") if bias is not None else None,
                                         _dev(skip, "skip") if skip is not None else None, out.data_ptr(), Cin, cout,
                                         D, H, W, stride, ACT_RELU if relu else ACT_NONE, _stream(x_cl)), "cds_conv3d_sbf_f32")
    return out


def deconv3d_k3s2(x: Tensor, wpk: Tensor, bias: Optional[Tensor], relu: bool = True,
                  skip: Optional[Tensor] = None) -> Tensor:
    Cin, D, H, W = x.shape
    if wpk.shape[0] != Cin or wpk.shape[1] != 27:
        raise ValueError("deconv3d_k3s2: packed weight must be [Cin,27,Cout]")
    Cout = wpk.shape[2]
    out = torch.empty((Cout, 2 * D, 2 * H, 2 * W), dtype=torch.float32, device=x.device)
    if skip is not None and skip.shape != out.shape:
        raise ValueError("deconv3d_k3s2: residual shape mismatch")
    check(_lib.load().cds_deconv3d_k3s2_f32(_dev(x, "x"), _dev(wpk, "weight"),
                                            _dev(bias, "bias") if bias is not None else None,
                                            _dev(skip, "skip") if skip is not None else None, out.data_ptr(), Cin, Cout,
                                            D, H, W, ACT_RELU if relu else ACT_NONE, _stream(x)),
          "cds_deconv3d_k3s2_f32")
    return out


def conv2d(x: Tensor, wpk: Tensor, bias: Optional[Tensor], cout: int, k: int, stride: int = 1, pad: int = 0,
           act: int = ACT_NONE, out: Optional[Tensor] = None, in_affine: Optional[Tensor] = None) -> Tensor:
    N, Cin, H, W = x.shape
    if in_affine is not None and tuple(in_affine.shape) != (N, Cin, 3):
        raise ValueError(f"conv2d: in_affine must be [{N},{Cin},3], got {tuple(in_affine.shape)}")
    coutp = (cout + 7) // 8 * 8
    if tuple(wpk.shape) != (Cin, k * k, coutp):
        raise ValueError(f"conv2d: packed weight must be [{Cin},{k * k},{coutp}], got {tuple(wpk.shape)}")
    Ho, Wo = (H + 2 * pad - k) // stride + 1, (W + 2 * pad - k) // stride + 1
    if out is None:
        out = torch.empty((N, cout, Ho, Wo), dtype=torch.float32, device=x.device)
    elif out.numel() != N * cout * Ho * Wo:
        raise ValueError("conv2d: bad output buffer")
    check(_lib.load().cds_conv2d_affine_f32(_dev(x, "x"), _dev(in_affine, "in_affine") if in_affine is not None else None,
                                            _dev(wpk, "weight"), _dev(bias, "bias") if bias is not None else None,
                                            _dev(out, "out"), N, Cin, cout, H, W, k, stride, pad, act, _stream(x)),
          "cds_conv2d_affine_f32")
    return out


USE_CONV2D_MFMA = os.environ.get("CDS_CONV2D_MFMA", "1") != "0"
USE_CONV2D_SBF = os.environ.get("CDS_CONV_EXACT", "0") != "1" and os.environ.get("CDS_CONV2D_SBF", "1") != "0"


def conv2d_c16_supported(x: Tensor) -> bool:
    return USE_CONV2D_MFMA and x.dim() == 4 and x.shape[1] == 16 and x.shape[3] % 4 == 0 and x.shape[3] >= 4


def conv2d_k3_c16(x: Tensor, wcl: Tensor, bias: Optional[Tensor], act: int = ACT_RELU, head_w: Optional[Tensor] = None,
                  head_b: Optional[Tensor] = None) -> Tensor:
    N, C, H, W = x.shape
    if C != 16 or tuple(wcl.shape) != (9, 16, 16) or W % 4:
        raise ValueError(f"conv2d_k3_c16: need x [N,16,H,W%4==0] and wcl [9,16,16], got {tuple(x.shape)}, {tuple(wcl.shape)}")
    if (head_w is None) != (head_b is None) or (head_w is not None and (head_w.numel() != 16 or head_b.numel() != 1)):
        raise ValueError("conv2d_k3_c16: head_w [16] and head_b [1] go together")
    out = torch.empty((N, H, W) if head_w is not None else (N, 16, H, W), dtype=torch.float32, device=x.device)
    check(_lib.load().cds_conv2d_k3_c16_f32(_dev(x, "x"), _dev(wcl, "weight_cl"), _dev(bias, "bias") if bias is not None else None,
                                            _dev(head_w, "head_w") if head_w is not None else None,
                                            _dev(head_b, "head_b") if head_b is not None else None,
                                            _dev(out, "out"), N, H, W, act, _stream(x)), "cds_conv2d_k3_c16_f32")
    return out


def conv2d_k3_relu_sbf(x: Tensor, wsplit: Tensor, bias: Optional[Tensor], head_w: Optional[Tensor] = None,
                       head_b: Optional[Tensor] = None) -> Tensor:
    N, C, H, W = x.shape
    if C % 8 or W % 4:
        raise ValueError(f"conv2d_k3_relu_sbf: need Cin % 8 == 0 and W % 4 == 0, got {tuple(x.shape)}")
    if (head_w is None) != (head_b is None) or (head_w is not None and (head_w.numel() != 16 or head_b.numel() != 1)):
        raise ValueError("conv2d_k3_relu_sbf: head_w [16] and head_b [1] go together")
    out = torch.empty((N, H, W) if head_w is not None else (N, 16, H, W), dtype=torch.float32, device=x.device)
    check(_lib.load().cds_conv2d_k3_relu_sbf_f32(_dev(x, "x"), wsplit.data_ptr(), _dev(bias, "bias") if bias is not None else None,
                                                 _dev(head_w, "head_w") if head_w is not None else None,
                                                 _dev(head_b, "head_b") if head_b is not None else None,
                                                 _dev(out, "out"), N, C, H, W, _stream(x)), "cds_conv2d_k3_relu_sbf_f32")
    return out


def dynconv_sbf_supported(Cin: int, co3: int, ksizes, W: int, fused: bool = False) -> bool:
    nb, nblk = len(ksizes), (co3 + 15) // 16
    worth = fused or max(ksizes) >= 5 or Cin >= 32
    return (USE_CONV2D_SBF and worth and Cin % 8 == 0 and W % 4 == 0 and all(k in (1, 3, 5, 7) for k in ksizes)
            and (nb, nblk) in ((3, 1), (3, 2), (2, 1), (2, 2), (2, 3)))


def split_pack_dynconv(ws, f16: bool = False):
    Co3, Cin = ws[0].shape[:2]
    rounds, nblk = Cin // 8, (Co3 + 15) // 16
    parts = []
    for w in ws:
        k = w.shape[-1]
        nks = (k * k + 3) // 4
        taps = torch.zeros((nblk * 16, rounds, nks * 4, 8), dtype=torch.float32, device=w.device)
        taps[:Co3, :, :k * k] = w.detach().float().reshape(Co3, rounds, 8, k * k).permute(0, 1, 3, 2)
        parts.append(taps.reshape(nblk, 16, rounds, nks, 4, 8).permute(2, 3, 0, 4, 1, 5).reshape(rounds, nks, nblk, 64, 8))
    a = torch.cat(parts, dim=1)
    return _split2_f16(a) if f16 else _split3(a)


def split_pack_conv00(ws, f16: bool = False):
    parts = []
    for w in ws:
        co3, cin, k, _ = w.shape
        if cin != 3 or co3 > 16:
            raise ValueError("split_pack_conv00: weights must be [<=16, 3, k, k]")
        np_ = (k + 1) // 2
        npairs, nks = k * np_, (k * np_ + 3) // 4
        wp = torch.zeros((co3, 3, k, 2 * np_), dtype=torch.float32, device=w.device)
        wp[..., :k] = w.detach().float()
        t = torch.zeros((16, nks * 4, 2, 4), dtype=torch.float32, device=w.device)
        t[:co3, :npairs, :, :3] = wp.reshape(co3, 3, k, np_, 2).permute(0, 2, 3, 4, 1).reshape(co3, npairs, 2, 3)
        parts.append(t.reshape(16, nks, 4, 8).permute(1, 2, 0, 3).reshape(nks, 64, 8))
    a = torch.cat(parts, dim=0)
    return _split2_f16(a) if f16 else _split3(a)


def conv00_cl(imgs: Tensor, wsplit: Tensor, bias: Optional[Tensor], w1: Tensor, b1: Tensor, w2: Tensor, epipoles: Tensor,
              temperature: float, n_shared: int = 1, stats_slope: float = 0.1, in_bound: Optional[Tensor] = None,
              w_inv_scale: float = 1.0):
    S, C, H, W = imgs.shape
    N = S + n_shared - 1
    if C != 3 or tuple(epipoles.shape) != (N, 2) or n_shared < 1:
        raise ValueError(f"conv00_cl: need imgs [S,3,H,W] and epipoles [S + n_shared - 1, 2], got {tuple(imgs.shape)}, {tuple(epipoles.shape)}")
    if wsplit.dtype != torch.int16 or wsplit.numel() != 26 * 3 * 64 * 8:
        raise ValueError("conv00_cl: wsplit must come from split_pack_conv00 (kernel sizes 3, 7, 11)")
    if bias is not None and tuple(bias.shape) != (3, 11):
        raise ValueError("conv00_cl: bias must be [3, 11]")
    dev = imgs.device
    epipoles = geo(epipoles, dev, "epipoles")
    lib = _lib.load()
    out = torch.empty((N, H, W, 8), dtype=torch.float32, device=dev)
    nc = torch.empty((N, H, W), dtype=torch.float32, device=dev)
    partial = torch.empty((N, lib.cds_dynconv_cl_parts(H, W), 8, 2), dtype=torch.float64, device=dev)
    if in_bound is not None:
        check(lib.cds_conv00_cl_sf16_f32(_dev(imgs, "imgs"), wsplit.data_ptr(), _dev(bias, "bias") if bias is not None else None,
                                         _dev(w1, "w1"), _dev(b1, "b1"), _dev(w2, "w2"), _dev(epipoles, "epipoles"), float(temperature),
                                         out.data_ptr(), nc.data_ptr(), partial.data_ptr(), N, n_shared, H, W, _dev(in_bound, "in_bound"),
                                         float(w_inv_scale), _stream(imgs)), "cds_conv00_cl_sf16_f32")
    else:
        check(lib.cds_conv00_cl_f32(_dev(imgs, "imgs"), wsplit.data_ptr(), _dev(bias, "bias") if bias is not None else None, _dev(w1, "w1"),
                                    _dev(b1, "b1"), _dev(w2, "w2"), _dev(epipoles, "epipoles"), float(temperature), out.data_ptr(),
                                    nc.data_ptr(), partial.data_ptr(), N, n_shared, H, W, _stream(imgs)), "cds_conv00_cl_f32")
    stats, affine = _reduce_records(partial, N, 8, H, W, stats_slope)
    return out, nc, stats, affine


def dynconv_branches_sbf(x: Tensor, wsplit: Tensor, bias: Optional[Tensor], co3: int, ksizes, out: Optional[Tensor] = None,
                         in_affine: Optional[Tensor] = None) -> Tensor:
    N, Cin, H, W = x.shape
    K = len(ksizes)
    if in_affine is not None and tuple(in_affine.shape) != (N, Cin, 3):
        raise ValueError(f"dynconv_branches_sbf: in_affine must be [{N},{Cin},3]")
    if out is None:
        out = torch.empty((K, N, co3, H, W), dtype=torch.float32, device=x.device)
    elif tuple(out.shape) != (K, N, co3, H, W):
        raise ValueError("dynconv_branches_sbf: bad output buffer")
    if bias is not None and tuple(bias.shape) != (K, co3):
        raise ValueError("dynconv_branches_sbf: bias must be [K, co3]")
    import ctypes
    ks = (ctypes.c_int * K)(*[int(k) for k in ksizes])
    check(_lib.load().cds_dynconv_branches_sbf_f32(_dev(x, "x"), _dev(in_affine, "in_affine") if in_affine is not None else None,
                                                   wsplit.data_ptr(), _dev(bias, "bias") if bias is not None else None,
                                                   _dev(out, "out"), N, Cin, co3, H, W, ks, K, _stream(x)),
          "cds_dynconv_branches_sbf_f32")
    return out


def dynconv_fused_sbf(x: Tensor, wsplit: Tensor, bias: Optional[Tensor], cout: int, ksizes, w1: Tensor, b1: Tensor, w2: Tensor,
                      epipoles: Tensor, temperature: float, stats_slope: float, in_affine: Optional[Tensor] = None):
    N, Cin, H, W = x.shape
    K = len(ksizes)
    if in_affine is not None and tuple(in_affine.shape) != (N, Cin, 3):
        raise ValueError(f"dynconv_fused_sbf: in_affine must be [{N},{Cin},3]")
    if bias is not None and tuple(bias.shape) != (K, cout + 3):
        raise ValueError("dynconv_fused_sbf: bias must be [K, cout + 3]")
    if tuple(epipoles.shape) != (N, 2):
        raise ValueError("dynconv_fused_sbf: epipoles must be [N,2]")
    dev = x.device
    epipoles = geo(epipoles, dev, "epipoles")
    lib = _lib.load()
    out = torch.empty((N, cout, H, W), dtype=torch.float32, device=dev)
    nc = torch.empty((N, H, W), dtype=torch.float32, device=dev)
    parts = lib.cds_dynconv_fused_parts(H, W)
    partial = torch.empty((N, parts, cout, 2), dtype=torch.float64, device=dev)
    stats = torch.empty((N, cout, 2), dtype=torch.float64, device=dev)
    affine = torch.empty((N, cout, 3), dtype=torch.float32, device=dev)
    import ctypes
    ks = (ctypes.c_int * K)(*[int(k) for k in ksizes])
    check(lib.cds_dynconv_fused_sbf_f32(_dev(x, "x"), _dev(in_affine, "in_affine") if in_affine is not None else None,
                                        wsplit.data_ptr(), _dev(bias, "bias") if bias is not None else None, _dev(w1, "w1"),
                                        _dev(b1, "b1"), _dev(w2, "w2"), _dev(epipoles, "epipoles"), float(temperature),
                                        out.data_ptr(), nc.data_ptr(), partial.data_ptr(), N, Cin, cout, H, W, ks, K, _stream(x)),
          "cds_dynconv_fused_sbf_f32")
    check(lib.cds_instnorm_reduce_f32(partial.data_ptr(), parts, stats.data_ptr(), affine.data_ptr(), N, cout, H, W,
                                      float(stats_slope), _stream(out)), "cds_instnorm_reduce_f32")
    return out, nc, stats, affine


def conv2d_fpn(coarse: Tensor, skip: Tensor, wpk: Tensor, cout: int, coarse_affine: Optional[Tensor] = None,
               skip_affine: Optional[Tensor] = None, stats_slope: Optional[float] = None):
    N, Ca, hc, wc = coarse.shape
    Nb, Cb, H, W = skip.shape
    if Nb != N or H != 2 * hc or W != 2 * wc:
        raise ValueError(f"conv2d_fpn: skip {tuple(skip.shape)} is not twice coarse {tuple(coarse.shape)}")
    coutp = (cout + 7) // 8 * 8
    if tuple(wpk.shape) != (Ca + Cb, 1, coutp):
        raise ValueError(f"conv2d_fpn: packed weight must be [{Ca + Cb},1,{coutp}], got {tuple(wpk.shape)}")
    for a, c, nm in ((coarse_affine, Ca, "coarse_affine"), (skip_affine, Cb, "skip_affine")):
        if a is not None and tuple(a.shape) != (N, c, 3):
            raise ValueError(f"conv2d_fpn: {nm} must be [{N},{c},3], got {tuple(a.shape)}")
    dev = skip.device
    lib = _lib.load()
    out = torch.empty((N, cout, H, W), dtype=torch.float32, device=dev)
    parts = lib.cds_fpn_stats_parts(H, W) if stats_slope is not None else 0
    partial = torch.empty((N, parts, cout, 2), dtype=torch.float64, device=dev) if parts else None
    check(lib.cds_conv2d_fpn_f32(_dev(coarse, "coarse"),
                                 _dev(coarse_affine, "coarse_affine") if coarse_affine is not None else None,
                                 _dev(skip, "skip"), _dev(skip_affine, "skip_affine") if skip_affine is not None else None,
                                 _dev(wpk, "weight"), _dev(out, "out"), partial.data_ptr() if parts else None,
                                 N, Ca, Cb, cout, H, W, _stream(skip)), "cds_conv2d_fpn_f32")
    if stats_slope is None:
        return out
    stats = torch.empty((N, cout, 2), dtype=torch.float64, device=dev)
    affine = torch.empty((N, cout, 3), dtype=torch.float32, device=dev)
    check(lib.cds_instnorm_reduce_f32(partial.data_ptr(), parts, stats.data_ptr(), affine.data_ptr(), N, cout, H, W,
                                      float(stats_slope), _stream(skip)), "cds_instnorm_reduce_f32")
    return out, affine


def instnorm_affine(x: Tensor, slope: float = 0.1) -> Tensor:
    N, C, H, W = x.shape
    aff = torch.empty((N, C, 3), dtype=torch.float32, device=x.device)
    stats = torch.empty((2 * N * C,), dtype=torch.float64, device=x.device)
    check(_lib.load().cds_instnorm_affine_f32(_dev(x, "x"), aff.data_ptr(), stats.data_ptr(), N, C, H, W, float(slope),
                                              _stream(x)), "cds_instnorm_affine_f32")
    return aff


def dynconv_blend(branches: Tensor, w1: Tensor, b1: Tensor, w2: Tensor, epipoles: Tensor,
                  temperature: float, n_shared: int = 1, stats_slope: Optional[float] = None):
    K, nslots, C3, H, W = branches.shape
    N = nslots + n_shared - 1
    cout = C3 - 3
    if tuple(epipoles.shape) != (N, 2) or n_shared < 1:
        raise ValueError("dynconv_blend: epipoles must be [N,2]")
    dev = branches.device
    epipoles = geo(epipoles, dev, "epipoles")
    out = torch.empty((N, cout, H, W), dtype=torch.float32, device=dev)
    nc = torch.empty((N, H, W), dtype=torch.float32, device=dev)
    lib = _lib.load()
    if stats_slope is None:
        check(lib.cds_dynconv_blend_shared_f32(_dev(branches, "branches"), _dev(w1, "w1"), _dev(b1, "b1"), _dev(w2, "w2"),
                                               _dev(epipoles, "epipoles"), float(temperature), out.data_ptr(),
                                               nc.data_ptr(), N, K, cout, H, W, n_shared, _stream(out)),
              "cds_dynconv_blend_shared_f32")
        return out, nc
    parts = lib.cds_blend_stats_parts(H, W)
    partial = torch.empty((N, parts, cout, 2), dtype=torch.float64, device=dev)
    stats = torch.empty((N, cout, 2), dtype=torch.float64, device=dev)
    affine = torch.empty((N, cout, 3), dtype=torch.float32, device=dev)
    check(lib.cds_dynconv_blend_stats_f32(_dev(branches, "branches"), _dev(w1, "w1"), _dev(b1, "b1"), _dev(w2, "w2"),
                                          _dev(epipoles, "epipoles"), float(temperature), out.data_ptr(), nc.data_ptr(),
                                          partial.data_ptr(), N, K, cout, H, W, n_shared, _stream(out)),
          "cds_dynconv_blend_stats_f32")
    check(lib.cds_instnorm_reduce_f32(partial.data_ptr(), parts, stats.data_ptr(), affine.data_ptr(), N, cout, H, W,
                                      float(stats_slope), _stream(out)), "cds_instnorm_reduce_f32")
    return out, nc, stats, affine


def instnorm_apply(x: Tensor, stats: Tensor, act: int, out_hwc: bool = False) -> Tensor:
    N, C, H, W = x.shape
    if stats.dtype != torch.float64 or tuple(stats.shape) != (N, C, 2):
        raise ValueError(f"instnorm_apply: stats must be float64 [{N},{C},2], got {stats.dtype} {tuple(stats.shape)}")
    out = torch.empty((N, H, W, C) if out_hwc else (N, C, H, W), dtype=torch.float32, device=x.device)
    check(_lib.load().cds_instnorm_apply_f32(_dev(x, "x"), _dev64(stats, "stats"), out.data_ptr(), N, C, H, W, act,
                                             1 if out_hwc else 0, _stream(x)), "cds_instnorm_apply_f32")
    return out


def instnorm_act(x: Tensor, act: int, out_hwc: bool = False) -> Tensor:
# ... 443 lines not shown
```

include/cds_mvsnet_hip.h:

```cpp
#ifndef CDS_MVSNET_HIP_H
#define CDS_MVSNET_HIP_H

#ifdef __cplusplus
extern "C" {
#endif

#define CDS_EINVAL (-1000)
#define CDS_MAX_VIEWS 8
#define CDS_MAX_IMAGES 16
#define CDS_STAGE_STATE_WORDS 2080

#define CDS_ACT_NONE 0
#define CDS_ACT_RELU 1
#define CDS_ACT_LEAKY01 2
#define CDS_ACT_SIGMOID 3
#define CDS_ACT_ACCUM 16
#define CDS_ACT_TANH 4

#define CDS_AGG_ACCUMULATE 1
#define CDS_AGG_NORMALIZE 2
#define CDS_AGG_CHANNELS_LAST 4
#define CDS_AGG_FAST_POSITIONS 8
#define CDS_WARP_FAST_POSITIONS CDS_AGG_FAST_POSITIONS

int cds_version(void);

int cds_chw_to_hwc_f32(const float* src_chw, float* dst_hwc, int C, int h, int w, void* stream);

int cds_stage_inputs_f32(const float* const* ref_feas, const float* const* src_feas, const float* const* ref_nc,
                         const float* const* ref_ncsum, const float* const* src_ncsum, float* ref_chw_out, float* src_hwc_out,
                         float* ref_nc_out, float* nc_mean_out, float* state, int V, int C, int h, int w, void* stream);

int cds_homo_warp_f32(const float* src_hwc, const float* mat, const float* hyp, float* out,
                      int C, int D, int h, int w, int hyp_per_pixel, void* stream);

int cds_warp_entropy_f32(const float* ref_chw, const float* src_hwc, const float* mats,
                         const float* hyp, float* entropy, int V, int C, int D, int h, int w,
                         int hyp_per_pixel, void* stream);
int cds_warp_entropy_flags_f32(const float* ref_chw, const float* src_hwc, const float* mats,
                               const float* hyp, float* entropy, int V, int C, int D, int h, int w,
                               int hyp_per_pixel, int flags, void* stream);

int cds_warp_aggregate_f32(const float* ref_chw, const float* src_hwc, const float* vis_w,
                           const float* mats, const float* hyp, float* volume, float* vis_sum,
                           int V, int C, int D, int h, int w, int hyp_per_pixel, int flags,
                           void* stream);

int cds_warp_entropy_window_f32(const float* ref_chw, const float* src_hwc, const float* mats, const float* hyp,
                                float* entropy, int V, int C, int D, int h, int w, int hs, int y_off, int flags, void* stream);
int cds_warp_aggregate_window_f32(const float* ref_chw, const float* src_hwc, const float* vis_w, const float* mats,
                                  const float* hyp, float* volume, float* vis_sum, int V, int C, int D, int h, int w, int hs,
                                  int y_off, int flags, void* stream);

int cds_warp_aggregate_bwd_f32(const float* ref_chw, const float* src_hwc, const float* vis_w,
                               const float* mats, const float* hyp, const float* grad_volume,
                               float* grad_ref, float* grad_src_hwc, float* grad_vis, int V, int C, int D,
                               int h, int w, int hyp_per_pixel, void* stream);
int cds_volume_finish_f32(const float* volume_sum, const float* gt_sum, const float* vis, int V, int C, int D, int hw, float* volume,
                          float* feat_distance, void* stream);
int cds_volume_finish_bwd_f32(const float* g_volume, const float* g_feat_distance, const float* volume_sum, const float* gt_sum,
                              const float* vis, int V, int C, int D, int hw, float* g_volume_sum, float* g_gt_sum, float* g_vis,
                              float* scratch, void* stream);

int cds_volume_normalize_f32(float* volume, const float* vis_sum, int C, int D, int hw, void* stream);

int cds_volume_normalize_cl_f32(float* volume, const float* vis_sum, int C, int D, int hw, void* stream);

int cds_softargmin_conf_f32(const float* prob_pre, const float* hyp, float* depth, float* conf,
                            float* prob, int D, int h, int w, int hyp_per_pixel, void* stream);

int cds_depth_hypotheses_f32(const float* prev_depth, float* out, int D, int hp, int wp, int H, int W,
                             int scale, const float* interval, const float* depth_range, void* stream);

int cds_depth_planes_f32(float* out, int D, int h, int w, const float* depth_range, void* stream);

int cds_conv3d_k3_f32(const float* x, const float* weight, const float* bias, const float* skip,
                      float* out, int Cin, int Cout, int D, int H, int W, int stride, int act,
                      void* stream);

int cds_conv3d_k3_cl_f32(const float* x, const float* weight_cl, const float* bias, const float* skip,
                         float* out, int Cin, int Cout, int D, int H, int W, int act, void* stream);

#define CDS_SBF_PAIR 101
int cds_conv3d_sbf_f32(const float* x, const void* weight_split, const float* bias, const float* skip, float* out,
                       int Cin, int Cout, int D, int H, int W, int stride, int act, void* stream);
int cds_conv3d_sf16_f32(const float* x, const void* weight_split, const float* bias, float* out, int Cin, int Cout, int D, int H, int W,
                        int stride, int act, const float* in_bound, float w_inv_scale, float* out_bound, void* stream);


int cds_deconv3d_sbf_f32(const float* x, const void* weight_split, const float* bias, const float* skip, float* out,
                         int Cin, int Cout, int D, int H, int W, int act, int out_planar, void* stream);

int cds_deconv3d_zm_f32(const float* x, const void* weight_cls, const float* bias, const float* skip, float* out,
                        int Cin, int Cout, int D, int H, int W, int act, void* stream);
int cds_deconv3d_sf16_f32(const float* x, const void* weight_split, const float* bias, const float* skip, float* out, int Cin, int Cout,
                          int D, int H, int W, int act, const float* in_bound, float w_inv_scale, float* out_bound, void* stream);
int cds_deconv3d_zm_sf16_f32(const float* x, const void* weight_cls, const float* bias, const float* skip, float* out, int Cin, int Cout,
                             int D, int H, int W, int act, const float* in_bound, float w_inv_scale, float* out_bound, void* stream);


int cds_deconv_prob_zm_f32(const float* x, const void* weight_split, const float* bias, const float* skip,
                           const float* prob_table, float* out, int D, int H, int W, void* stream);
int cds_deconv_prob_zm_sf16_f32(const float* x, const void* weight_split, const float* bias, const float* skip, const float* prob_table,
                                float* out, int D, int H, int W, const float* in_bound, float w_inv_scale, void* stream);


int cds_deconv3d_k3s2_f32(const float* x, const float* weight, const float* bias, const float* skip,
                          float* out, int Cin, int Cout, int D, int H, int W, int act, void* stream);

int cds_conv2d_f32(const float* x, const float* weight, const float* bias, float* out, int N, int Cin,
                   int Cout, int H, int W, int k, int stride, int pad, int act, void* stream);
int cds_conv2d_affine_f32(const float* x, const float* in_affine, const float* weight, const float* bias, float* out,
                          int N, int Cin, int Cout, int H, int W, int k, int stride, int pad, int act, void* stream);

int cds_conv2d_k3_c16_f32(const float* x, const float* weight_cl, const float* bias, const float* head_w,
                          const float* head_b, float* out, int N, int H, int W, int act, void* stream);

int cds_dynconv_branches_sbf_f32(const float* x, const float* in_affine, const void* weight_split, const float* bias,
                                 float* out, int N, int Cin, int Co3, int H, int W, const int* ksizes, int nb, void* stream);

int cds_dynconv_fused_sbf_f32(const float* x, const float* in_affine, const void* weight_split, const float* bias,
                              const float* w1, const float* b1, const float* w2, const float* epipoles,
                              float temperature, float* out, float* norm_curv, double* partial, int N, int Cin, int Cout,
                              int H, int W, const int* ksizes, int nb, void* stream);
int cds_dynconv_fused_parts(int H, int W);

int cds_conv2d_k3_relu_sbf_f32(const float* x, const void* weight_split, const float* bias, const float* head_w,
                               const float* head_b, float* out, int N, int Cin, int H, int W, void* stream);

int cds_fpn_stats_parts(int H, int W);
int cds_conv2d_fpn_f32(const float* coarse, const float* coarse_affine, const float* skip, const float* skip_affine,
                       const float* weight, float* out, float* partial, int N, int Ca, int Cb, int Cout, int H, int W,
                       void* stream);

int cds_dynconv_blend_f32(const float* branches, const float* w1, const float* b1, const float* w2,
                          const float* epipoles, float temperature, float* out, float* norm_curv,
                          int N, int K, int Cout, int H, int W, void* stream);
int cds_dynconv_blend_shared_f32(const float* branches, const float* w1, const float* b1, const float* w2,
                                 const float* epipoles, float temperature, float* out, float* norm_curv, int N,
                                 int K, int Cout, int H, int W, int n_shared, void* stream);

int cds_blend_stats_parts(int H, int W);
int cds_dynconv_blend_stats_f32(const float* branches, const float* w1, const float* b1, const float* w2,
                                const float* epipoles, float temperature, float* out, float* norm_curv,
                                float* partial, int N, int K, int Cout, int H, int W, int n_shared, void* stream);
int cds_instnorm_reduce_f32(const float* partial, int parts, float* stats, float* affine, int N, int C, int H, int W,
                            float slope, void* stream);
int cds_instnorm_apply_f32(const float* x, const float* stats, float* out, int N, int C, int H, int W, int act,
                           int out_hwc, void* stream);

int cds_instnorm_act_f32(const float* x, float* out, float* stats, int N, int C, int H, int W, int act,
                         int out_hwc, void* stream);
int cds_instnorm_affine_f32(const float* x, float* affine, float* stats, int N, int C, int H, int W, float slope,
                            void* stream);

int cds_debug_poison_lds(unsigned pattern);

int cds_dynconv_cl_parts(int H, int W);
int cds_dynconv_cl_f32(const float* x, const float* in_affine, const void* weight_split, const float* bias, const float* w1,
                       const float* b1, const float* w2, const float* epipoles, float temperature, float* out,
                       float* norm_curv, double* partial, int N, int C, int H, int W, const int* ksizes, int nb, void* stream);
int cds_dynconv_cl_sf16_f32(const float* x, const float* in_affine, const void* weight_split, const float* bias, const float* w1,
                            const float* b1, const float* w2, const float* epipoles, float temperature, float* out, float* norm_curv,
                            double* partial, int N, int C, int H, int W, const int* ksizes, int nb, float x_bound, float w_inv_scale,
                            void* stream);

int cds_conv00_cl_f32(const float* x, const void* weight_split, const float* bias, const float* w1, const float* b1, const float* w2,
                      const float* epipoles, float temperature, float* out, float* norm_curv, double* partial, int N, int n_shared,
                      int H, int W, void* stream);
int cds_conv00_cl_sf16_f32(const float* x, const void* weight_split, const float* bias, const float* w1, const float* b1, const float* w2,
                           const float* epipoles, float temperature, float* out, float* norm_curv, double* partial, int N, int n_shared,
                           int H, int W, const float* in_bound, float w_inv_scale, void* stream);

int cds_blend_cl_parts(int H, int W);
int cds_dynconv_blend_cl_f32(const float* branches, const float* w1, const float* b1, const float* w2, const float* epipoles,
                             float temperature, float* out, float* norm_curv, double* partial, int N, int K, int Cout, int H, int W,
                             int n_shared, void* stream);
int cds_conv2d_k3s2_cl_f32(const float* x, const float* in_affine, const float* weight, float* out, int N, int Cin, int Cout, int H,
                           int W, void* stream);
int cds_conv2d_k3s2_cl_sf16_f32(const float* x, const float* in_affine, const void* weight_split, float* out, int N, int Cin, int Cout,
                                int H, int W, float x_bound, float w_inv_scale, void* stream);

int cds_fpn_cl_parts(int H, int W);
int cds_conv2d_fpn_cl_f32(const float* coarse, const float* coarse_affine, const float* skip, const float* skip_affine,
                          const float* weight, float* out, double* partial, int N, int Ca, int Cb, int Cout, int H, int W,
                          void* stream);
int cds_vis_layer1_cl_f32(const float* entropy, const float* ref_nc, const float* weight, const float* bias, float* out, int V, int H,
                          int W, void* stream);
int cds_conv2d_k3_relu_cl_f32(const float* x, const void* weight_split, const float* bias, const float* head_w, const float* head_b,
                              float* out, int N, int Cin, int H, int W, void* stream);
int cds_instnorm_stats_cl_parts(int H, int W);
int cds_instnorm_stats_cl_f32(const float* x, double* partial, int N, int C, int H, int W, void* stream);
int cds_instnorm_apply_cl_f32(const float* x, const double* stats, float* out_cl, float* out_chw, int N, int C, int H, int W, int act,
                              int n_chw, int cl_from, void* stream);

int cds_depth_fusion_f32(const float* ref_depth, const float* ref_conf, const float* src_depths,
                         const float* src_confs, const float* cams, float* fused, float* mask, float* points,
                         float* view_masks, int V, int h, int w, const float* prob_thresh_host,
                         float dist_thresh, float depth_thresh, float view_thresh, void* stream);

int cds_curvature_stats_f32(const float* a, const float* b, const float* c, float* nc_sum, float* nc_abs, int n,
                            void* stream);
int cds_curvature_stats_bwd_f32(const float* a, const float* b, const float* c, const float* g_sum, const float* g_abs, float* ga,
                                float* gb, float* gc, int n, void* stream);
int cds_pair_mean_f32(const float* x, float* out, int V, int n, void* stream);
int cds_view_mean_f32(const float* x, float* out, int V, int n, void* stream);

int cds_depth_affine_f32(const float* depth, float* out, int n, const float* depth_range, void* stream);
int cds_deconv2d_k3s2_f32(const float* x, const float* weight, const float* bias, float* out, int Cin, int Cout,
                          int H, int W, int act, void* stream);
int cds_refine_finish_f32(const float* d_norm, const float* res, float* out, int h, int w, const float* depth_range,
                          void* stream);

int cds_bn3d_stats_f32(const float* x, double* sums, int B, int C, long long V, void* stream);
int cds_bn3d_norm_f32(const float* y, const double* sums, const float* gamma, const float* beta, double n, double eps, float momentum,
                      float* running_mean, float* running_var, const float* skip, float* out, float* scale, float* shift, double* mean,
                      double* invstd, int B, int C, long long V, int relu, void* stream);
int cds_bn3d_bwd_reduce_f32(const float* dout, const float* y, const float* scale, const float* shift, double* sums, int B,
                            int C, long long V, int relu, void* stream);
int cds_bn3d_bwd_norm_f32(const float* dout, const float* y, const float* scale, const float* shift, const double* sums,
                          const double* mean, const double* invstd, double n, float* dy, float* dgamma, float* dbeta, int B, int C,
                          long long V, int relu, void* stream);
int cds_conv3d_wgrad_f32(const float* g, const float* xin, float* dw, int B, int Ca, int Cb, int Do, int Ho, int Wo, int Di,
                         int Hi, int Wi, int stride, void* stream);

int cds_bn3d_norm_bound_f32(const float* y, const double* sums, const float* gamma, const float* beta, double n, double eps,
                            float momentum, float* running_mean, float* running_var, const float* skip, float* out, float* scale,
                            float* shift, double* mean, double* invstd, int B, int C, long long V, int relu, float* out_bound,
                            void* stream);
int cds_bn3d_bwd_norm_bound_f32(const float* dout, const float* y, const float* scale, const float* shift, const double* sums,
                                const double* mean, const double* invstd, double n, float* dy, float* dgamma, float* dbeta, int B, int C,
                                long long V, int relu, float* dy_bound, void* stream);
int cds_absmax_bound_f32(const float* x, long long n, float* bound, void* stream);
int cds_sf16_pack_conv3d_f32(const float* w, void* fwd, void* dgrad, float* w_inv, int A, int B, int mode, void* stream);
int cds_conv3d_k3_sf16_f32(const float* x, const void* wpk, const float* w_inv, const float* x_bound, float* y, int B, int C, int M,
                           int Di, int Hi, int Wi, int mode, void* stream);
int cds_conv3d_wgrad_sf16_f32(const float* g, const float* xin, const float* g_bound, const float* x_bound, float* dw, int B, int Ca,
                              int Cb, int Do, int Ho, int Wo, int Di, int Hi, int Wi, int stride, void* stream);

int cds_conv2d_wgrad_f32(const float* g, const float* x, float* dw, int N, int Co, int Cin, int Ho, int Wo, int H, int W, int k,
                         int stride, int pad, void* stream);
int cds_conv2d_dgrad_s2_f32(const float* g, const float* w, float* gx, int N, int Co, int Cin, int Ho, int Wo, int H, int W,
                            void* stream);
int cds_instnorm_bwd_f32(const float* gz, const float* y, const double* stats, double* sums, float* gy, int N, int C, int H, int W,
                         int act, int scratch_zeroed, void* stream);
int cds_dynconv_bn_stats_f32(const float* branches, const float* epipoles, const float* w1, double* mom, float* mean, float* rstd,
                             float* running_mean, float* running_var, int N, int G, int K, int Cout, int H, int W, float eps,
                             float momentum, int use_batch, int scratch_zeroed, void* stream);
int cds_dynconv_blend_train_f32(const float* branches, const float* epipoles, const float* w1, const float* w2, const float* gamma,
                                const float* beta, const float* mean, const float* rstd, float temperature, float* out,
                                float* norm_curv, int N, int G, int K, int Cout, int H, int W, void* stream);
int cds_dynconv_blend_bwd_f32(const float* branches, const float* epipoles, const float* w1, const float* w2, const float* gamma,
                              const float* beta, const float* mean, const float* rstd, float temperature, const float* gy,
                              const float* gnc, float* gbr, double* sums, double* dw1, int N, int G, int K, int Cout, int H, int W,
                              int use_batch, int scratch_zeroed, void* stream);
int cds_f32_to_bf16(const float* src, unsigned short* dst, long long n, void* stream);
int cds_instnorm_act_b16_f32(const float* y, unsigned short* y16, float* out32, unsigned short* out16, double* stats, int N, int C,
                             int H, int W, int act, int strict, void* stream);
int cds_conv2d_wgrad_xb16_f32(const float* g, const unsigned short* x, float* dw, int N, int Co, int Cin, int Ho, int Wo, int H, int W,
                              int k, int stride, int pad, void* stream);
int cds_instnorm_bwd_yb16_f32(const float* gz, const unsigned short* y, const unsigned short* z16, const double* stats, double* sums,
                              float* gy, int N, int C, int H, int W, int act, int scratch_zeroed, void* stream);
int cds_dynconv_bn_stats_b16_f32(const unsigned short* branches, const float* epipoles, const float* w1, double* mom, float* mean,
                                 float* rstd, float* running_mean, float* running_var, int N, int G, int K, int Cout, int H, int W,
                                 float eps, float momentum, int use_batch, int scratch_zeroed, void* stream);
int cds_dynconv_blend_train_b16_f32(const unsigned short* branches, const float* epipoles, const float* w1, const float* w2,
                                    const float* gamma, const float* beta, const float* mean, const float* rstd, float temperature,
                                    float* out, float* norm_curv, int N, int G, int K, int Cout, int H, int W, void* stream);
int cds_dynconv_blend_bwd_b16_f32(const unsigned short* branches, const float* epipoles, const float* w1, const float* w2,
                                  const float* gamma, const float* beta, const float* mean, const float* rstd, float temperature,
                                  const float* gy, const float* gnc, float* gbr, double* sums, double* dw1, int N, int G, int K,
                                  int Cout, int H, int W, int use_batch, int scratch_zeroed, void* stream);
int cds_pack_conv2d_f32(const float* wa, const float* wb, float* fwd, float* dgrad, int Ca, int Cb, int Cin, int k, void* stream);
int cds_pack_conv3d_f32(const float* w, float* fwd, float* dgrad, int A, int B, int mode, void* stream);
int cds_softargmin_bwd_f32(const float* prob_pre, const float* hyp, const float* gdepth, float* gpre, int D, int h, int w,
                           int hyp_per_pixel, void* stream);
int cds_dynconv_bwd_finish_f32(const double* sums, const double* dw1, int G, int K, float* out, void* stream);

int cds_loss_records(long long elements);
int cds_loss_stage_f32(const float* depth, const float* gt, const float* mask, const float* norm_curv, const float* dist,
                       const float* target, const float* interval, int B, int hw, int Dp, double* recA, double* recB, void* stream);
int cds_loss_final_f32(const double* const* recA, const double* const* recB, const long long* pixels, const int* Dp, const float* weight,
                       const int* has_curv, int n_stages, float* total, float* depth_loss, double* scalars, void* stream);
int cds_loss_stage_bwd_f32(const float* depth, const float* gt, const float* mask, const float* dist, const float* target,
                           const float* interval, const float* gtotal, const double* scalars, float weight, int B, int hw, int Dp,
                           float* gdepth, float* gnc, float* gdist, void* stream);
int cds_feat_target_f32(const float* hyp, const float* gt, const float* di, float scale, float thresh, int B, int D, int hw,
                        float* target, void* stream);

int cds_bn_running_update_f32(const float* batch_mean, const float* batch_var, const float* group_weights, float keep, int G, int C,
                              float* running_mean, float* running_var, void* stream);

int cds_grid_hash_log2_slots(long long n_keys);
int cds_grid_keys_f32(const float* points, long long n, const float* frame_host, long long* keys, void* stream);
int cds_grid_hash_build(const long long* keys, long long n_keys, long long n_fine, long long* table_keys, int* table_vals,
                        int log2_slots, void* stream);
int cds_nn_query_f32(const float* query, const long long* order, long long m, const float* pts, const int* cell_start,
                     const long long* cell_keys, const int* coarse_start, const long long* table_keys, const int* table_vals,
                     int log2_slots, const float* frame_host, float max_dist, float* dist, void* stream);
int cds_thin_round_f32(const float* pts, const int* cell_start, long long n, const long long* table_keys, const int* table_vals,
                       int log2_slots, const float* frame_host, float min_dist, unsigned char* state, int* undecided,
                       void* stream);

int cds_gipuma_tiles(long long n);
int cds_gipuma_prob_filter_f32(const float* depths, const float* confs, const unsigned char* rgb8, int V, int h, int w,
                               const float* prob_thresh_host, float* depth_out, unsigned* rgb_out, void* stream);
int cds_gipuma_fuse_view_f32(const float* depths, const unsigned* rgb, const float* views, const float* fb, int r, int V, int h,
                             int w, float depth_min, float depth_max, float disp_thresh, int num_consistent, unsigned char* used,
                             unsigned char* emit, unsigned* records, void* stream);
int cds_gipuma_scan(const unsigned char* emit, int tiles, int* tile_count, int* tile_off, int* total, void* stream);
int cds_gipuma_compact_f32(const unsigned char* emit, const unsigned* records, const int* tile_off, int tiles, int hw,
                           float* points, unsigned* colors, int* ref_view, void* stream);

#define CDS_COLMAP_SCORE_QUANTUM_LOG2 80
#define CDS_COLMAP_SCORE_MAX_LIMBS 28
int cds_colmap_score_quantum_log2(void);
int cds_colmap_score_limbs(double theta0, double sigma1, double sigma2);
int cds_colmap_pair_scores_f64(const long long* pair_off, const long long* ptr, const int* img, const int* cnt,
                               const double* xyz, const double* centres, long long P, long long T, int N, double theta0,
                               double sigma1, double sigma2, int limbs, long long* acc, void* stream);
int cds_colmap_obs_depth_f64(const int* obs_img, const long long* obs_pt, const double* xyz, const double* zrow, long long n,
                             double* z, void* stream);
int cds_colmap_depth_ranges_f64(const double* z_sorted, const long long* obs_ptr, const int* num_min, const int* num_max,
                                int N, double* out, void* stream);

#ifdef __cplusplus
}
#endif
#endif
```

Measured before the change: 184.7 depth-maps/s.

## Make zmg conv3d kernel persistent, walking multiple tiles per workgroup

The zmg 3D conv kernel now launches at most one workgroup per CU (queried from the device). Each workgroup loops over several tile/z-segment units, and the producer waves prefetch the next unit's initial planes while the current one finishes. The segment-count cost model uses the real CU count instead of a hardcoded 256. The change also adds a plan query API, an optional out tensor for conv3d_sbf, 32-bit source offsets guarded by a size check, and an atomic-max bound publish that skips redundant atomics. The goal is to cut tail effects and per-workgroup setup and LDS-priming cost, at the price of longer-running workgroups and less dynamic load balancing.

Result: no change. 184.3 depth-maps/s (-0.2%).

```diff
diff --git a/cds_mvsnet_amd/_lib.py b/cds_mvsnet_amd/_lib.py
--- a/cds_mvsnet_amd/_lib.py
+++ b/cds_mvsnet_amd/_lib.py
@@ -44,6 +44,7 @@
     "cds_conv3d_k3_cl_f32": [P, P, P, P, P, I, I, I, I, I, I, P],
     "cds_conv3d_sbf_f32": [P, P, P, P, P, I, I, I, I, I, I, I, P],
     "cds_conv3d_sf16_f32": [P, P, P, P, I, I, I, I, I, I, I, P, F, P, P],
+    "cds_conv3d_zmg_plan": [I, I, I, I, I, I, I, P, P],
     "cds_deconv3d_sbf_f32": [P, P, P, P, P, I, I, I, I, I, I, I, P],
     "cds_deconv3d_sf16_f32": [P, P, P, P, P, I, I, I, I, I, I, P, F, P, P],
     "cds_deconv3d_zm_sf16_f32": [P, P, P, P, P, I, I, I, I, I, I, P, F, P, P],
@@ -144,6 +145,8 @@
     "cds_colmap_depth_ranges_f64": [P, P, P, P, I, P, P],
 }
 
+OPTIONAL = {"cds_conv3d_zmg_plan"}
+
 _lib = None
 
 
@@ -167,6 +170,8 @@
         try:
             fn = getattr(lib, name)
         except AttributeError as e:
+            if name in OPTIONAL and os.environ.get("CDS_MVSNET_LIB"):
+                continue
             raise CdsLibraryError(f"{LIB_PATH} does not export {name}") from e
         fn.argtypes = argtypes
         fn.restype = c_int
diff --git a/cds_mvsnet_amd/csrc/cds_common.hpp b/cds_mvsnet_amd/csrc/cds_common.hpp
--- a/cds_mvsnet_amd/csrc/cds_common.hpp
+++ b/cds_mvsnet_amd/csrc/cds_common.hpp
@@ -13,6 +13,7 @@
 int cds_conv3d_zmg_dispatch(const float* x, const void* wsp, const float* bias, float* out, int Cin, int Cout, int D, int H, int W,
                             int stride, int pair, int act, hipStream_t st, const float* in_bound = nullptr, float w_inv = 1.f,
                             float* out_bound = nullptr);
+int cds_conv3d_zmg_plan_dispatch(int Cin, int Cout, int D, int H, int W, int stride, int pair, int f16, int* plan);
 
 using cds_f4 = float __attribute__((ext_vector_type(4)));
 
diff --git a/cds_mvsnet_amd/csrc/conv3d_sbf.hip b/cds_mvsnet_amd/csrc/conv3d_sbf.hip
--- a/cds_mvsnet_amd/csrc/conv3d_sbf.hip
+++ b/cds_mvsnet_amd/csrc/conv3d_sbf.hip
@@ -869,6 +869,17 @@
   return CDS_EINVAL;
 }
 
+extern "C" int cds_conv3d_zmg_plan(int Cin, int Cout, int D, int H, int W, int stride, int f16, int* workgroups, int* units_per_workgroup) {
+  if (!workgroups || !units_per_workgroup || Cin < 8 || (Cin % 8) || Cout < 4 || (Cout % 4) || Cout > 64 || D < 1 || H < 1 || W < 1 ||
+      (stride != 1 && stride != 2 && stride != CDS_SBF_PAIR) || (stride == CDS_SBF_PAIR && Cout != 8))
+    return CDS_EINVAL;
+  int plan[2] = {0, 0};
+  const int r = cds_conv3d_zmg_plan_dispatch(Cin, Cout, D, H, W, stride == CDS_SBF_PAIR ? 1 : stride, stride == CDS_SBF_PAIR, f16, plan);
+  *workgroups = r == 0 ? plan[0] : 0;
+  *units_per_workgroup = r == 0 ? plan[1] : 0;
+  return r;
+}
+
 extern "C" int cds_deconv3d_sf16_f32(const float* x, const void* weight_split, const float* bias, const float* skip, float* out, int Cin,
                                      int Cout, int D, int H, int W, int act, const float* in_bound, float w_inv_scale, float* out_bound,
                                      void* stream) {
diff --git a/cds_mvsnet_amd/csrc/conv3d_zmg.hip b/cds_mvsnet_amd/csrc/conv3d_zmg.hip
--- a/cds_mvsnet_amd/csrc/conv3d_zmg.hip
+++ b/cds_mvsnet_amd/csrc/conv3d_zmg.hip
@@ -50,6 +50,21 @@
   static constexpr int PT = PW * 64, PPT = (NITEM + PT - 1) / PT;
 };
 
+__device__ __forceinline__ int zmg_per_unit(int v) {
+  asm volatile("" : "+v"(v));
+  return v;
+}
+
+__device__ __forceinline__ void zmg_publish_bound(float amax, float* slot) {
+#pragma unroll
+  for (int o = 32; o > 0; o >>= 1) amax = fmaxf(amax, __shfl_xor(amax, o));
+  if (__lane_id() == 0 && slot) {
+    unsigned int* u = reinterpret_cast<unsigned int*>(slot);
+    const unsigned int mine = __float_as_uint(amax);
+    if (mine > __hip_atomic_load(u, __ATOMIC_RELAXED, __HIP_MEMORY_SCOPE_AGENT)) atomicMax(u, mine);
+  }
+}
+
 template <class Cfg>
 __global__ __launch_bounds__(Cfg::THREADS, 1) void conv3d_zmg_kernel(const float* __restrict__ x, const uint4* __restrict__ wsp,
                                                                   const float* __restrict__ bias, float* __restrict__ out, int Cout,
@@ -63,18 +78,21 @@
   const float xs = F16 ? sf16_scale(in_bound[0]) : 1.0f;
   const float out_mul = F16 ? w_inv / xs : 1.0f;
   extern __shared__ __attribute__((aligned(16))) unsigned char lds[];
-  const int tid = threadIdx.x;
-  const int lane = tid & 63;
-  const int wave = __builtin_amdgcn_readfirstlane(tid >> 6);
+  const int lane = __lane_id();
+  const int wave = __builtin_amdgcn_readfirstlane(threadIdx.x >> 6);
   const int nseg = (Do + zseg - 1) / zseg;
-  int unit = cds_xcd_remap(blockIdx.x, gridDim.x);
-  const int seg = unit % nseg;
-  unit /= nseg;
-  const int tx_i = unit % tiles_x, ty_i = unit / tiles_x;
-  const int z0 = seg * zseg, z1 = min(Do, z0 + zseg);
-  const int nstages = (z1 - z0 + G - 1) / G;
-  const int gx0 = tx_i * Cfg::TXO * S - 1, gy0 = ty_i * Cfg::TYO * S - 1;
-  const int zin0 = S * z0 - 1;
+  const int nunits = tiles_x * tiles_y * nseg;
+  if ((int)blockIdx.x >= nunits) return;
+  const int nwalk = (nunits - 1 - (int)blockIdx.x) / (int)gridDim.x + 1;
+  auto unit_at = [&](int it, int& tx_i, int& ty_i, int& z0, int& z1) __attribute__((always_inline)) {
+    int unit = cds_xcd_remap(blockIdx.x + it * gridDim.x, nunits);
+    const int seg = unit % nseg;
+    unit /= nseg;
+    tx_i = unit % tiles_x;
+    ty_i = unit / tiles_x;
+    z0 = seg * zseg;
+    z1 = min(Do, z0 + zseg);
+  };
 
   if (wave >= Cfg::CW) {
 #ifndef CDS_ZMG_PPRIO
@@ -82,10 +100,8 @@
 #endif
     __builtin_amdgcn_s_setprio(CDS_ZMG_PPRIO);
     constexpr int PT = Cfg::PT, PPT = Cfg::PPT;
-    const int ptid = tid - Cfg::CW * 64;
+    const int ptid = (wave - Cfg::CW) * 64 + lane;
     int s_pl[PPT], s_dst[PPT];
-    long long s_off[PPT];
-    unsigned okmask = 0;
 #pragma unroll
     for (int h = 0; h < PPT; ++h) {
       const int p = h * PT + ptid;
@@ -93,17 +109,36 @@
       const int rd = t1 % RD, t2 = t1 / RD;
       const int row = t2 % Cfg::IY, pl = t2 / Cfg::IY;
       const int c = Cfg::DEINT ? (2 * (q % Cfg::IXH) + q / Cfg::IXH) : q;
-      const int gy = gy0 + row, gx = gx0 + c;
       const bool exists = p < Cfg::NITEM && c < Cfg::IX;
-      s_pl[h] = pl;
+      s_pl[h] = exists ? pl : -1;
       s_dst[h] = rd * Cfg::SLICEB + (row * Cfg::IXP + q) * POSB;
-      s_off[h] = ((long long)gy * W + gx) * Cin + rd * 8;
-      if (exists && (unsigned)gy < (unsigned)H && (unsigned)gx < (unsigned)W) okmask |= 1u << h;
-      if (!exists) s_pl[h] = -1;
     }
+    int gx0, gy0, zin0, nstages;
+    int s_off[PPT];
+    unsigned okmask;
+    auto set_unit = [&](int it) __attribute__((always_inline)) {
+      int tx_i, ty_i, z0, z1;
+      unit_at(it, tx_i, ty_i, z0, z1);
+      nstages = (z1 - z0 + G - 1) / G;
+      gx0 = tx_i * Cfg::TXO * S - 1;
+      gy0 = ty_i * Cfg::TYO * S - 1;
+      zin0 = S * z0 - 1;
+      okmask = 0;
+      const int upt = zmg_per_unit(ptid);
+#pragma unroll
+      for (int h = 0; h < PPT; ++h) {
+        const int p = h * PT + upt;
+        const int q = p % Cfg::IXP, t1 = p / Cfg::IXP;
+        const int rd = t1 % RD, row = (t1 / RD) % Cfg::IY;
+        const int c = Cfg::DEINT ? (2 * (q % Cfg::IXH) + q / Cfg::IXH) : q;
+        const int gy = gy0 + row, gx = gx0 + c;
+        s_off[h] = (gy * W + gx) * Cin + rd * 8;
+        if (s_pl[h] >= 0 && (unsigned)gy < (unsigned)H && (unsigned)gx < (unsigned)W) okmask |= 1u << h;
+      }
+    };
     const long long plane_elems = (long long)H * W * Cin;
     float4 va[2][PPT], vb[2][PPT];
-    auto issue = [&](int st, int set) {
+    auto issue = [&](int st, int set) __attribute__((always_inline)) {
       const int zn = zin0 + st * S * G + Cfg::NINIT;
 #pragma unroll
       for (int h = 0; h < PPT; ++h) {
@@ -114,7 +149,7 @@
         vb[set][h] = *reinterpret_cast<const float4*>(src + 4);
       }
     };
-    auto deposit = [&](int st, int set) {
+    auto deposit = [&](int st, int set) __attribute__((always_inline)) {
       const int slot0 = (st * S * G + Cfg::NINIT) % R;
 #pragma unroll
       for (int h = 0; h < PPT; ++h) {
@@ -125,37 +160,66 @@
         else split_store8(lds + slot * Cfg::PLANEB + s_dst[h], va[set][h], vb[set][h]);
       }
     };
-    for (int p = ptid; p < Cfg::NINIT * Cfg::IY * RD * Cfg::IXP; p += PT) {
-      const int q = p % Cfg::IXP, t1 = p / Cfg::IXP;
-      const int rd = t1 % RD, t2 = t1 / RD;
-      const int row = t2 % Cfg::IY, pl = t2 / Cfg::IY;
-      const int c = Cfg::DEINT ? (2 * (q % Cfg::IXH) + q / Cfg::IXH) : q;
-      const int gz = zin0 + pl, gy = gy0 + row, gx = gx0 + c;
-      const bool ok = c < Cfg::IX && (unsigned)gz < (unsigned)D && (unsigned)gy < (unsigned)H && (unsigned)gx < (unsigned)W;
-      const float* __restrict__ src = ok ? x + (((long long)gz * H + gy) * W + gx) * Cin + rd * 8 : g_zmg_zeros;
-      if (F16)
-        split_store8_f16(lds + pl * Cfg::PLANEB + rd * Cfg::SLICEB + (row * Cfg::IXP + q) * POSB, *reinterpret_cast<const float4*>(src),
-                         *reinterpret_cast<const float4*>(src + 4), xs);
-      else
-        split_store8(lds + pl * Cfg::PLANEB + rd * Cfg::SLICEB + (row * Cfg::IXP + q) * POSB, *reinterpret_cast<const float4*>(src),
-                     *reinterpret_cast<const float4*>(src + 4));
-    }
-    issue(0, 0);
-    if (nstages > 1) issue(1, 1);
-    deposit(0, 0);
-    if (nstages > 2) issue(2, 0);
-    __syncthreads();
-    for (int st = 0; st < nstages; st += 2) {
-      if (st + 1 < nstages) {
+    constexpr int NIN = Cfg::NINIT * Cfg::IY * RD * Cfg::IXP, PPI = (NIN + PT - 1) / PT;
+    float4 ia[PPI], ib[PPI];
+    auto issue_init = [&]() __attribute__((always_inline)) {
+      const int upt = zmg_per_unit(ptid);
+#pragma unroll
+      for (int h = 0; h < PPI; ++h) {
+        const int p = h * PT + upt;
+        const int q = p % Cfg::IXP, t1 = p / Cfg::IXP;
+        const int rd = t1 % RD, t2 = t1 / RD;
+        const int row = t2 % Cfg::IY, pl = t2 / Cfg::IY;
+        const int c = Cfg::DEINT ? (2 * (q % Cfg::IXH) + q / Cfg::IXH) : q;
+        const int gz = zin0 + pl, gy = gy0 + row, gx = gx0 + c;
+        const bool ok = p < NIN && c < Cfg::IX && (unsigned)gz < (unsigned)D && (unsigned)gy < (unsigned)H && (unsigned)gx < (unsigned)W;
+        const float* __restrict__ src = ok ? x + (((long long)gz * H + gy) * W + gx) * Cin + rd * 8 : g_zmg_zeros;
+        ia[h] = *reinterpret_cast<const float4*>(src);
+        ib[h] = *reinterpret_cast<const float4*>(src + 4);
+      }
+    };
+    auto deposit_init = [&]() __attribute__((always_inline)) {
+      const int upt = zmg_per_unit(ptid);
+#pragma unroll
+      for (int h = 0; h < PPI; ++h) {
+        const int p = h * PT + upt;
+        if (p >= NIN) continue;
+        const int q = p % Cfg::IXP, t1 = p / Cfg::IXP;
+        const int rd = t1 % RD, t2 = t1 / RD;
+        const int row = t2 % Cfg::IY, pl = t2 / Cfg::IY;
+        unsigned char* dst = lds + pl * Cfg::PLANEB + rd * Cfg::SLICEB + (row * Cfg::IXP + q) * POSB;
+        if (F16) split_store8_f16(dst, ia[h], ib[h], xs);
+        else split_store8(dst, ia[h], ib[h]);
+      }
+    };
+    auto prime = [&](int it) __attribute__((always_inline)) {
+      set_unit(it);
+      issue_init();
+      issue(0, 0);
+    };
+    prime(0);
+    for (int it = 0; it < nwalk; ++it) {
+      const int nst = nstages;
+      const bool more = it + 1 < nwalk;
+      deposit_init();
+      if (nst > 1) issue(1, 1);
+      deposit(0, 0);
+      if (nst > 2) issue(2, 0);
+      __syncthreads();
+      int st = 0;
+      for (; st + 2 < nst; st += 2) {
         deposit(st + 1, 1);
-        if (st + 3 < nstages) issue(st + 3, 1);
-      }
-      __syncthreads();
-      if (st + 1 >= nstages) break;
-      if (st + 2 < nstages) {
+        if (st + 3 < nst) issue(st + 3, 1);
+        __syncthreads();
         deposit(st + 2, 0);
-        if (st + 4 < nstages) issue(st + 4, 0);
-      }
+        if (st + 4 < nst) issue(st + 4, 0);
+        __syncthreads();
+      }
+      if (st + 1 < nst) {
+        deposit(st + 1, 1);
+        __syncthreads();
+      }
+      if (more) prime(it + 1);
       __syncthreads();
     }
     return;
@@ -166,14 +230,11 @@
 #endif
   __builtin_amdgcn_s_setprio(CDS_ZMG_CPRIO);
   const int k = wave % Cfg::KSPL, mbi = (wave / Cfg::KSPL) % Cfg::MBS, part = wave / (Cfg::KSPL * Cfg::MBS);
-  const int j = lane & 15, g = lane >> 4;
 #ifdef CDS_ZMG_NOSKEW
   const bool late = false;
 #else
   const bool late = Cfg::CW == 8 && wave >= 4;
 #endif
-  const int lane_base = k * Cfg::RPW * Cfg::SLICEB + (part * Cfg::ROWS * S * Cfg::IXP + j) * POSB +
-                        (PAIR ? (((g & 1) * 2 + (g >> 1)) & 1) * Cfg::IXH * POSB + ((((g & 1) * 2 + (g >> 1))) >> 1) * POSB : 0);
   constexpr int RPW = Cfg::RPW;
   const int mbg = (Cfg::YS > 1 ? blockIdx.y * Cfg::MBS : 0) + mbi;
   BV wres[RPW * KS][NT];
@@ -187,160 +248,184 @@
     }
   }
   float amax = 0.f;
-  const int co = PAIR ? 4 * (g & 1) : mbg * 16 + 4 * g;
-  const float4 bv = (bias && co < Cout) ? *reinterpret_cast<const float4*>(bias + co) : make_float4(0.f, 0.f, 0.f, 0.f);
-  constexpr int XW = PAIR ? 32 : 16;
-  const int oy0 = ty_i * Cfg::TYO + part * Cfg::ROWS;
-  const int ox0 = tx_i * Cfg::TXO + (PAIR ? 2 * j + (g >> 1) : j);
-  float* const obase = out + ((size_t)((size_t)z0 * Ho + oy0) * Wo + ox0) * Cout + co;
-  bool lane_ok[Cfg::XT];
-#pragma unroll
-  for (int xt = 0; xt < Cfg::XT; ++xt) lane_ok[xt] = ox0 + xt * XW < Wo && co < Cout;
-  auto store_tile = [&](int n, int st, const f32x4& a) {
-    const int i = n % G, rx = n / G, xt = rx % Cfg::XT, r = rx / Cfg::XT;
-    if (z0 + st * G + i >= z1 || oy0 + r >= Ho) return;
-    if (!lane_ok[xt]) return;
-    float4 o = F16 ? make_float4(a.x * out_mul + bv.x, a.y * out_mul + bv.y, a.z * out_mul + bv.z, a.w * out_mul + bv.w)
-                   : make_float4(a.x + bv.x, a.y + bv.y, a.z + bv.z, a.w + bv.w);
-    if (act == CDS_ACT_RELU) {
-      o.x = fmaxf(o.x, 0.f); o.y = fmaxf(o.y, 0.f); o.z = fmaxf(o.z, 0.f); o.w = fmaxf(o.w, 0.f);
+  const int cob = PAIR ? 4 * ((lane >> 4) & 1) : mbg * 16 + 4 * (lane >> 4);
+  const float4 bv = (bias && cob < Cout) ? *reinterpret_cast<const float4*>(bias + cob) : make_float4(0.f, 0.f, 0.f, 0.f);
+  for (int it = 0; it < nwalk; ++it) {
+    int tx_i, ty_i, z0, z1;
+    unit_at(it, tx_i, ty_i, z0, z1);
+    const int nstages = (z1 - z0 + G - 1) / G;
+    const int ul = zmg_per_unit(lane);
+    const int j = ul & 15, g = ul >> 4;
+    const int co = PAIR ? 4 * (g & 1) : mbg * 16 + 4 * g;
+    const int lane_base = k * Cfg::RPW * Cfg::SLICEB + (part * Cfg::ROWS * S * Cfg::IXP + j) * POSB +
+                          (PAIR ? (((g & 1) * 2 + (g >> 1)) & 1) * Cfg::IXH * POSB + ((((g & 1) * 2 + (g >> 1))) >> 1) * POSB : 0);
+    constexpr int XW = PAIR ? 32 : 16;
+    const int oy0 = ty_i * Cfg::TYO + part * Cfg::ROWS;
+    const int ox0 = tx_i * Cfg::TXO + (PAIR ? 2 * j + (g >> 1) : j);
+    float* const obase = out + ((size_t)((size_t)z0 * Ho + oy0) * Wo + ox0) * Cout + co;
+    bool lane_ok[Cfg::XT];
+#pragma unroll
+    for (int xt = 0; xt < Cfg::XT; ++xt) lane_ok[xt] = ox0 + xt * XW < Wo && co < Cout;
+    auto store_tile = [&](int n, int st, const f32x4& a) {
+      const int i = n % G, rx = n / G, xt = rx % Cfg::XT, r = rx / Cfg::XT;
+      if (z0 + st * G + i >= z1 || oy0 + r >= Ho) return;
+      if (!lane_ok[xt]) return;
+      float4 o = F16 ? make_float4(a.x * out_mul + bv.x, a.y * out_mul + bv.y, a.z * out_mul + bv.z, a.w * out_mul + bv.w)
+                     : make_float4(a.x + bv.x, a.y + bv.y, a.z + bv.z, a.w + bv.w);
+      if (act == CDS_ACT_RELU) {
+        o.x = fmaxf(o.x, 0.f); o.y = fmaxf(o.y, 0.f); o.z = fmaxf(o.z, 0.f); o.w = fmaxf(o.w, 0.f);
+      }
+      if (F16) amax = fmaxf(fmaxf(amax, fmaxf(fabsf(o.x), fabsf(o.y))), fmaxf(fabsf(o.z), fabsf(o.w)));
+      sbf_store4(obase + ((size_t)((size_t)(st * G + i) * Ho + r) * Wo + xt * XW) * Cout, o);
+    };
+    unsigned char* xch = lds + Cfg::RINGB;
+    constexpr int NH = NTW / 2;
+    f32x4 acc[NTW];
+    constexpr bool KEEP4 = Cfg::RPW == 1;
+    f32x4 keep[Cfg::KSPL == 2 ? NH : Cfg::NFIN];
+    auto store_tile_rt = [&](int n, int st, const f32x4& a) {
+      const int i = n % G, rx = n / G, xt = rx % Cfg::XT, r = rx / Cfg::XT;
+      if (z0 + st * G + i >= z1 || oy0 + r >= Ho) return;
+      if (!(ox0 + xt * XW < Wo && co < Cout)) return;
+      float4 o = F16 ? make_float4(a.x * out_mul + bv.x, a.y * out_mul + bv.y, a.z * out_mul + bv.z, a.w * out_mul + bv.w)
+                     : make_float4(a.x + bv.x, a.y + bv.y, a.z + bv.z, a.w + bv.w);
+      if (act == CDS_ACT_RELU) {
+        o.x = fmaxf(o.x, 0.f); o.y = fmaxf(o.y, 0.f); o.z = fmaxf(o.z, 0.f); o.w = fmaxf(o.w, 0.f);
+      }
+      if (F16) amax = fmaxf(fmaxf(amax, fmaxf(fabsf(o.x), fabsf(o.y))), fmaxf(fabsf(o.z), fabsf(o.w)));
+      sbf_store4(obase + ((size_t)((size_t)(st * G + i) * Ho + r) * Wo + xt * XW) * Cout, o);
+    };
+    const int xgrp = (wave / Cfg::KSPL) * NTW;
+    auto finish = [&](int sp) {
+      if (Cfg::KSPL == 2) {
+        const unsigned char* src = xch + (sp & 1) * Cfg::XCH1 + ((wave ^ 1) * NH) * 1024 + ul * 16;
+#pragma unroll
+        for (int m = 0; m < NH; ++m) {
+          const f32x4 o = *reinterpret_cast<const f32x4*>(src + m * 1024);
+          store_tile(k * NH + m, sp, k == 0 ? keep[m] + o : o + keep[m]);
+        }
+      } else if (Cfg::KSPL == 4) {
+#pragma unroll
+        for (int jf = 0; jf < Cfg::NFIN; ++jf) {
+          const int n = jf * 4 + k;
+          if (n >= NTW) continue;
+          const unsigned char* src = xch + (sp & 1) * Cfg::XCH1 + ((xgrp + n) * 4) * 1024 + ul * 16;
+          f32x4 total = KEEP4 && k == 0 ? keep[jf] : *reinterpret_cast<const f32x4*>(src);
+#pragma unroll
+          for (int kk = 1; kk < 4; ++kk) total = total + (KEEP4 && kk == k ? keep[jf] : *reinterpret_cast<const f32x4*>(src + kk * 1024));
+          store_tile_rt(n, sp, total);
+        }
+      } else {
+#pragma unroll
+        for (int n = 0; n < NTW; ++n) store_tile(n, sp, acc[n]);
+      }
+    };
+    __syncthreads();
+    for (int st = 0; st < nstages; ++st) {
+      if (late && st > 0) finish(st - 1);
+      int vpl[PAIR ? Cfg::NRES : 1];
+      int vaddr[PAIR ? 1 : KS][PAIR ? 1 : G];
+      {
+        int sl[Cfg::NRES];
+        int slot = (st * S * G) % R;
+#pragma unroll
+        for (int u = 0; u < Cfg::NRES; ++u) {
+          sl[u] = slot * Cfg::PLANEB;
+          slot = slot + 1 >= R ? slot + 1 - R : slot + 1;
+        }
+        if (PAIR) {
+#pragma unroll
+          for (int u = 0; u < Cfg::NRES; ++u) vpl[u] = lane_base + sl[u];
+        } else {
+#pragma unroll
+          for (int t = 0; t < KS; ++t)
+#pragma unroll
+            for (int i = 0; i < G; ++i) {
+              const int o0 = sl[S * i + Cfg::tap_kz(t, 0)] + Cfg::tap_off(t, 0), o1 = sl[S * i + Cfg::tap_kz(t, 1)] + Cfg::tap_off(t, 1);
+              const int o2 = sl[S * i + Cfg::tap_kz(t, 2)] + Cfg::tap_off(t, 2), o3 = sl[S * i + Cfg::tap_kz(t, 3)] + Cfg::tap_off(t, 3);
+              vaddr[t][i] = lane_base + (g == 0 ? o0 : (g == 1 ? o1 : (g == 2 ? o2 : o3)));
+            }
+        }
+      }
+      constexpr int NGRP = NTW / NG, NS = RPW * KS * NGRP;
+      constexpr int PF = Cfg::PF;
+      BV bd[PF + 1][NG][NT];
+      auto load_b = [&](int buf, int ss) {
+        const int t = (ss / NGRP) % KS, rr = ss / (NGRP * KS), grp = ss % NGRP;
+#pragma unroll
+        for (int q = 0; q < NG; ++q) {
+          const int n = grp * NG + q, i = n % G, rx = n / G, xt = rx % Cfg::XT, r = rx / Cfg::XT;
+          const unsigned char* b = lds + (PAIR ? vpl[PAIR ? S * i + t / 3 : 0] + (t % 3) * Cfg::IXP * POSB : vaddr[PAIR ? 0 : t][PAIR ? 0 : i]) +
+                                   (r * S * Cfg::IXP + xt * 16) * POSB + rr * Cfg::SLICEB;
+          bd[buf][q][0].u = *reinterpret_cast<const uint4*>(b);
+          bd[buf][q][1].u = *reinterpret_cast<const uint4*>(b + 16);
+          if (!F16) bd[buf][q][NT - 1].u = *reinterpret_cast<const uint4*>(b + 32);
+        }
+      };
+      load_b(0, 0);
+      if (PF == 2 && NS > 1) load_b(1, 1);
+      __builtin_amdgcn_s_setprio(0);
+#pragma unroll
+      for (int t = 0; t < NTW; ++t) acc[t] = (f32x4){0.f, 0.f, 0.f, 0.f};
+#pragma unroll
+      for (int ss = 0; ss < NS; ++ss) {
+        const int t = ss / NGRP, grp = ss % NGRP, db = ss % (PF + 1);
+        if (ss + PF < NS) load_b((ss + PF) % (PF + 1), ss + PF);
+        __builtin_amdgcn_sched_barrier(0);
+  #ifndef CDS_ZMG_LAZYWAIT
+        if (ss + PF < NS) __builtin_amdgcn_s_waitcnt(0xC07F | ((PF * NT * NG) << 8));
+        else if (PF == 2 && ss + 1 < NS) __builtin_amdgcn_s_waitcnt(0xC07F | ((NT * NG) << 8));
+        else __builtin_amdgcn_s_waitcnt(0xC07F);
+        __builtin_amdgcn_sched_barrier(0);
+  #endif
+        if constexpr (F16) {
+          SF16_TERMS(acc, grp * NG, NG, wres[t], bd[db]);
+        } else {
+          SBF_TERMS(acc, grp * NG, NG, wres[t], bd[db]);
+        }
+      }
+      __builtin_amdgcn_s_setprio(CDS_ZMG_CPRIO);
+      if (Cfg::KSPL == 2) {
+        if (!late && st > 0) finish(st - 1);
+        unsigned char* dst = xch + (st & 1) * Cfg::XCH1 + (wave * NH) * 1024 + ul * 16;
+#pragma unroll
+        for (int m = 0; m < NH; ++m) {
+          *reinterpret_cast<f32x4*>(dst + m * 1024) = acc[(k ^ 1) * NH + m];
+          keep[m] = acc[k * NH + m];
+        }
+      } else if (Cfg::KSPL == 4) {
+        if (!late && st > 0) finish(st - 1);
+        unsigned char* dst = xch + (st & 1) * Cfg::XCH1 + (xgrp * 4 + k) * 1024 + ul * 16;
+#pragma unroll
+        for (int n = 0; n < NTW; ++n) {
+          if (KEEP4 && (n & 3) == k) keep[n >> 2] = acc[n];
+          else *reinterpret_cast<f32x4*>(dst + n * 4096) = acc[n];
+        }
+      } else if (!late) {
+        finish(st);
+      }
+      __syncthreads();
     }
-    if (F16) amax = fmaxf(fmaxf(amax, fmaxf(fabsf(o.x), fabsf(o.y))), fmaxf(fabsf(o.z), fabsf(o.w)));
-    sbf_store4(obase + ((size_t)((size_t)(st * G + i) * Ho + r) * Wo + xt * XW) * Cout, o);
-  };
-  unsigned char* xch = lds + Cfg::RINGB;
-  constexpr int NH = NTW / 2;
-  f32x4 acc[NTW];
-  constexpr bool KEEP4 = Cfg::RPW == 1;
-  f32x4 keep[Cfg::KSPL == 2 ? NH : Cfg::NFIN];
-  auto store_tile_rt = [&](int n, int st, const f32x4& a) {
-    const int i = n % G, rx = n / G, xt = rx % Cfg::XT, r = rx / Cfg::XT;
-    if (z0 + st * G + i >= z1 || oy0 + r >= Ho) return;
-    if (!(ox0 + xt * XW < Wo && co < Cout)) return;
-    float4 o = F16 ? make_float4(a.x * out_mul + bv.x, a.y * out_mul + bv.y, a.z * out_mul + bv.z, a.w * out_mul + bv.w)
-                   : make_float4(a.x + bv.x, a.y + bv.y, a.z + bv.z, a.w + bv.w);
-    if (act == CDS_ACT_RELU) {
-      o.x = fmaxf(o.x, 0.f); o.y = fmaxf(o.y, 0.f); o.z = fmaxf(o.z, 0.f); o.w = fmaxf(o.w, 0.f);
-    }
-    if (F16) amax = fmaxf(fmaxf(amax, fmaxf(fabsf(o.x), fabsf(o.y))), fmaxf(fabsf(o.z), fabsf(o.w)));
-    sbf_store4(obase + ((size_t)((size_t)(st * G + i) * Ho + r) * Wo + xt * XW) * Cout, o);
-  };
-  const int xgrp = (wave / Cfg::KSPL) * NTW;
-  auto finish = [&](int sp) {
-    if (Cfg::KSPL == 2) {
-      const unsigned char* src = xch + (sp & 1) * Cfg::XCH1 + ((wave ^ 1) * NH) * 1024 + lane * 16;
-#pragma unroll
-      for (int m = 0; m < NH; ++m) {
-        const f32x4 o = *reinterpret_cast<const f32x4*>(src + m * 1024);
-        store_tile(k * NH + m, sp, k == 0 ? keep[m] + o : o + keep[m]);
-      }
-    } else if (Cfg::KSPL == 4) {
-#pragma unroll
-      for (int jf = 0; jf < Cfg::NFIN; ++jf) {
-        const int n = jf * 4 + k;
-        if (n >= NTW) continue;
-        const unsigned char* src = xch + (sp & 1) * Cfg::XCH1 + ((xgrp + n) * 4) * 1024 + lane * 16;
-        f32x4 total = KEEP4 && k == 0 ? keep[jf] : *reinterpret_cast<const f32x4*>(src);
-#pragma unroll
-        for (int kk = 1; kk < 4; ++kk) total = total + (KEEP4 && kk == k ? keep[jf] : *reinterpret_cast<const f32x4*>(src + kk * 1024));
-        store_tile_rt(n, sp, total);
-      }
-    } else {
-#pragma unroll
-      for (int n = 0; n < NTW; ++n) store_tile(n, sp, acc[n]);
-    }
-  };
-  __syncthreads();
-  for (int st = 0; st < nstages; ++st) {
-    if (late && st > 0) finish(st - 1);
-    int vpl[PAIR ? Cfg::NRES : 1];
-    int vaddr[PAIR ? 1 : KS][PAIR ? 1 : G];
-    {
-      int sl[Cfg::NRES];
-      int slot = (st * S * G) % R;
-#pragma unroll
-      for (int u = 0; u < Cfg::NRES; ++u) {
-        sl[u] = slot * Cfg::PLANEB;
-        slot = slot + 1 >= R ? slot + 1 - R : slot + 1;
-      }
-      if (PAIR) {
-#pragma unroll
-        for (int u = 0; u < Cfg::NRES; ++u) vpl[u] = lane_base + sl[u];
-      } else {
-#pragma unroll
-        for (int t = 0; t < KS; ++t)
-#pragma unroll
-          for (int i = 0; i < G; ++i) {
-            const int o0 = sl[S * i + Cfg::tap_kz(t, 0)] + Cfg::tap_off(t, 0), o1 = sl[S * i + Cfg::tap_kz(t, 1)] + Cfg::tap_off(t, 1);
-            const int o2 = sl[S * i + Cfg::tap_kz(t, 2)] + Cfg::tap_off(t, 2), o3 = sl[S * i + Cfg::tap_kz(t, 3)] + Cfg::tap_off(t, 3);
-            vaddr[t][i] = lane_base + (g == 0 ? o0 : (g == 1 ? o1 : (g == 2 ? o2 : o3)));
-          }
-      }
-    }
-    constexpr int NGRP = NTW / NG, NS = RPW * KS * NGRP;
-    constexpr int PF = Cfg::PF;
-    BV bd[PF + 1][NG][NT];
-    auto load_b = [&](int buf, int ss) {
-      const int t = (ss / NGRP) % KS, rr = ss / (NGRP * KS), grp = ss % NGRP;
-#pragma unroll
-      for (int q = 0; q < NG; ++q) {
-        const int n = grp * NG + q, i = n % G, rx = n / G, xt = rx % Cfg::XT, r = rx / Cfg::XT;
-        const unsigned char* b = lds + (PAIR ? vpl[PAIR ? S * i + t / 3 : 0] + (t % 3) * Cfg::IXP * POSB : vaddr[PAIR ? 0 : t][PAIR ? 0 : i]) +
-                                 (r * S * Cfg::IXP + xt * 16) * POSB + rr * Cfg::SLICEB;
-        bd[buf][q][0].u = *reinterpret_cast<const uint4*>(b);
-        bd[buf][q][1].u = *reinterpret_cast<const uint4*>(b + 16);
-        if (!F16) bd[buf][q][NT - 1].u = *reinterpret_cast<const uint4*>(b + 32);
-      }
-    };
-    load_b(0, 0);
-    if (PF == 2 && NS > 1) load_b(1, 1);
-    __builtin_amdgcn_s_setprio(0);
-#pragma unroll
-    for (int t = 0; t < NTW; ++t) acc[t] = (f32x4){0.f, 0.f, 0.f, 0.f};
-#pragma unroll
-    for (int ss = 0; ss < NS; ++ss) {
-      const int t = ss / NGRP, grp = ss % NGRP, db = ss % (PF + 1);
-      if (ss + PF < NS) load_b((ss + PF) % (PF + 1), ss + PF);
-      __builtin_amdgcn_sched_barrier(0);
-#ifndef CDS_ZMG_LAZYWAIT
-      if (ss + PF < NS) __builtin_amdgcn_s_waitcnt(0xC07F | ((PF * NT * NG) << 8));
-      else if (PF == 2 && ss + 1 < NS) __builtin_amdgcn_s_waitcnt(0xC07F | ((NT * NG) << 8));
-      else __builtin_amdgcn_s_waitcnt(0xC07F);
-      __builtin_amdgcn_sched_barrier(0);
-#endif
-      if constexpr (F16) {
-        SF16_TERMS(acc, grp * NG, NG, wres[t], bd[db]);
-      } else {
-        SBF_TERMS(acc, grp * NG, NG, wres[t], bd[db]);
-      }
-    }
-    __builtin_amdgcn_s_setprio(CDS_ZMG_CPRIO);
-    if (Cfg::KSPL == 2) {
-      if (!late && st > 0) finish(st - 1);
-      unsigned char* dst = xch + (st & 1) * Cfg::XCH1 + (wave * NH) * 1024 + lane * 16;
-#pragma unroll
-      for (int m = 0; m < NH; ++m) {
-        *reinterpret_cast<f32x4*>(dst + m * 1024) = acc[(k ^ 1) * NH + m];
-        keep[m] = acc[k * NH + m];
-      }
-    } else if (Cfg::KSPL == 4) {
-      if (!late && st > 0) finish(st - 1);
-      unsigned char* dst = xch + (st & 1) * Cfg::XCH1 + (xgrp * 4 + k) * 1024 + lane * 16;
-#pragma unroll
-      for (int n = 0; n < NTW; ++n) {
-        if (KEEP4 && (n & 3) == k) keep[n >> 2] = acc[n];
-        else *reinterpret_cast<f32x4*>(dst + n * 4096) = acc[n];
-      }
-    } else if (!late) {
-      finish(st);
-    }
-    __syncthreads();
-  }
-  if (Cfg::KSPL >= 2 || late) finish(nstages - 1);
-  if (F16) sf16_publish_bound(amax, out_bound);
-}
-
-inline int zmg_pick_nseg(int cols, int Do, int G) {
+    if (Cfg::KSPL >= 2 || late) finish(nstages - 1);
+  }
+  if (F16) zmg_publish_bound(amax, out_bound);
+}
+
+inline int zmg_cu_count() {
+  static std::atomic<int> cached[64];
+  int d = 0;
+  (void)hipGetDevice(&d);
+  int v = cached[d & 63].load(std::memory_order_relaxed);
+  if (v > 0) return v;
+  if (hipDeviceGetAttribute(&v, hipDeviceAttributeMultiprocessorCount, d) != hipSuccess || v <= 0) {
+    (void)hipGetLastError();
+    v = 256;
+  }
+  cached[d & 63].store(v, std::memory_order_relaxed);
+  return v;
+}
+
+inline int zmg_pick_nseg(int cols, int Do, int G, int cus) {
   const int nseg_env = cds_env_int("CDS_ZMG_NSEG", 0);
   if (nseg_env > 0) return nseg_env;
   const int stages = cds_ceil_div(Do, G);
@@ -349,26 +434,44 @@
   for (int n = 1; n <= 32 && n <= stages; ++n) {
     const int per = cds_ceil_div(stages, n);
     if (n > 1 && per < 6) break;
-    const double cost = (double)cds_ceil_div(cols * cds_ceil_div(stages, per), 256) * (per + 2.5);
+    const double cost = (double)cds_ceil_div(cols * cds_ceil_div(stages, per), cus) * (per + 2.5);
     if (cost < best_cost - 1e-9) { best_cost = cost; best = n; }
   }
   return best;
 }
+
+thread_local int* t_zmg_plan = nullptr;
 
 template <class Cfg>
 int launch_zmg(const float* x, const void* wsp, const float* b, float* out, int Cout, int D, int H, int W, int act, hipStream_t st,
-               const float* in_bound = nullptr, float w_inv = 1.f, float* out_bound = nullptr, int min_wgs = 0) {
+               const float* in_bound = nullptr, float w_inv = 1.f, float* out_bound = nullptr, bool fill_chip = false) {
   constexpr int S = Cfg::S;
   const int Do = (D - 1) / S + 1, Ho = (H - 1) / S + 1, Wo = (W - 1) / S + 1;
   const int tx = cds_ceil_div(Wo, Cfg::TXO), ty = cds_ceil_div(Ho, Cfg::TYO);
-  int nseg = zmg_pick_nseg(tx * ty * Cfg::YS, Do, Cfg::G);
+  if ((long long)(H + 64) * (W + 64) * 8 * Cfg::RD > 0x7fffffffLL) return CDS_ZMG_UNSUPPORTED;
+  const int cus = zmg_cu_count();
+  int nseg = zmg_pick_nseg(tx * ty * Cfg::YS, Do, Cfg::G, cus);
   const int zseg = cds_ceil_div(cds_ceil_div(Do, nseg), Cfg::G) * Cfg::G;
   nseg = cds_ceil_div(Do, zseg);
-  if (min_wgs > 0 && tx * ty * nseg * Cfg::YS < min_wgs) return CDS_ZMG_UNSUPPORTED;
+  const int nunits = tx * ty * nseg;
+  if (fill_chip && nunits * Cfg::YS < cus) return CDS_ZMG_UNSUPPORTED;
+  const int persist = cds_env_int("CDS_ZMG_PERSIST", 1);
+  const int cap = cus / Cfg::YS > 0 ? cus / Cfg::YS : 1;
+  int wgs = nunits;
+  if (persist == 2 || (persist == 1 && nunits > cap)) {
+    wgs = nunits < cap ? nunits : cap;
+    const int wgs_env = cds_env_int("CDS_ZMG_PERSIST_WGS", 0);
+    if (wgs_env > 0) wgs = wgs_env;
+  }
+  if (t_zmg_plan) {
+    t_zmg_plan[0] = wgs * Cfg::YS;
+    t_zmg_plan[1] = cds_ceil_div(nunits, wgs);
+    return 0;
+  }
   auto kern = conv3d_zmg_kernel<Cfg>;
   static std::atomic<unsigned long long> lds_ok{0};
   if (int e_lds = cds_allow_lds(reinterpret_cast<const void*>(kern), Cfg::LDSB, lds_ok)) return e_lds;
-  hipLaunchKernelGGL(kern, dim3(tx * ty * nseg, Cfg::YS), dim3(Cfg::THREADS), Cfg::LDSB, st, x, reinterpret_cast<const uint4*>(wsp), b,
+  hipLaunchKernelGGL(kern, dim3(wgs, Cfg::YS), dim3(Cfg::THREADS), Cfg::LDSB, st, x, reinterpret_cast<const uint4*>(wsp), b,
                      out, Cout, D, H, W, Do, Ho, Wo, act, tx, ty, zseg, in_bound, w_inv, out_bound);
   return cds_launch_status();
 }
@@ -391,11 +494,11 @@
     if (stride == 2 && Cin == 16 && Cout == 32)
       return launch_zmg<ZG<2, 2, 2, false, 16, 4, 1, 1, 8, true>>(x, wsp, bias, out, Cout, D, H, W, act, st, in_bound, w_inv, out_bound);
     const int deep = cds_env_is("CDS_ZMG", '0') ? 0 : cds_env_int("CDS_ZMG_DEEP", 1);
-    const int min_wgs = deep == 2 ? 0 : 256;
+    const bool fill = deep != 2;
     if (deep > 0 && stride == 1 && Cin == 32 && Cout == 32)
-      return launch_zmg<ZG<1, 4, 2, false, 16, 4, 1, 1, 8, true, 1, 1, 2>>(x, wsp, bias, out, Cout, D, H, W, act, st, in_bound, w_inv, out_bound, min_wgs);
+      return launch_zmg<ZG<1, 4, 2, false, 16, 4, 1, 1, 8, true, 1, 1, 2>>(x, wsp, bias, out, Cout, D, H, W, act, st, in_bound, w_inv, out_bound, fill);
     if (deep > 0 && stride == 1 && Cin == 64 && Cout == 64)
-      return launch_zmg<ZG<1, 8, 4, false, 16, 2, 1, 1, 8, true, 2, 2>>(x, wsp, bias, out, Cout, D, H, W, act, st, in_bound, w_inv, out_bound, min_wgs);
+      return launch_zmg<ZG<1, 8, 4, false, 16, 2, 1, 1, 8, true, 2, 2>>(x, wsp, bias, out, Cout, D, H, W, act, st, in_bound, w_inv, out_bound, fill);
     return CDS_ZMG_UNSUPPORTED;
   }
   const bool off = cds_env_is("CDS_ZMG", '0');
@@ -414,3 +517,12 @@
   if (Cin == 16 && Cout == 32) return launch_zmg<ZG<2, 2, 2, false, 16, 4, 1, 1, 8>>(x, wsp, bias, out, Cout, D, H, W, act, st);
   return CDS_ZMG_UNSUPPORTED;
 }
+
+int cds_conv3d_zmg_plan_dispatch(int Cin, int Cout, int D, int H, int W, int stride, int pair, int f16, int* plan) {
+  static const float bound_tag = 0.f;
+  t_zmg_plan = plan;
+  const int r = cds_conv3d_zmg_dispatch(nullptr, nullptr, nullptr, nullptr, Cin, Cout, D, H, W, stride, pair, 0, nullptr,
+                                        f16 ? &bound_tag : nullptr, 1.f, nullptr);
+  t_zmg_plan = nullptr;
+  return r;
+}
diff --git a/cds_mvsnet_amd/ops.py b/cds_mvsnet_amd/ops.py
--- a/cds_mvsnet_amd/ops.py
+++ b/cds_mvsnet_amd/ops.py
@@ -652,13 +652,26 @@
                                                      (32, 32, 1), (32, 64, 2), (64, 64, 1))
 
 
+def conv3d_zmg_plan(cin: int, cout: int, D: int, H: int, W: int, stride: int = 1, f16: bool = True) -> Optional[Tuple[int, int]]:
+    import ctypes
+    wgs, per = ctypes.c_int(0), ctypes.c_int(0)
+    rc = _lib.load().cds_conv3d_zmg_plan(cin, cout, D, H, W, stride, int(f16), ctypes.byref(wgs), ctypes.byref(per))
+    if rc == 1:
+        return None
+    check(rc, "cds_conv3d_zmg_plan")
+    return wgs.value, per.value
+
+
 def conv3d_sbf(x_cl: Tensor, wsplit: Tensor, bias: Optional[Tensor], cout: int, stride: int = 1, relu: bool = True,
                skip: Optional[Tensor] = None, in_bound: Optional[Tensor] = None, w_inv_scale: float = 1.0,
-               out_bound: Optional[Tensor] = None) -> Tensor:
+               out_bound: Optional[Tensor] = None, out: Optional[Tensor] = None) -> Tensor:
     D, H, W, Cin = x_cl.shape
     sg = 1 if stride == SBF_PAIR else stride
     Do, Ho, Wo = (D - 1) // sg + 1, (H - 1) // sg + 1, (W - 1) // sg + 1
-    out = torch.empty((Do, Ho, Wo, cout), dtype=torch.float32, device=x_cl.device)
+    if out is None:
+        out = torch.empty((Do, Ho, Wo, cout), dtype=torch.float32, device=x_cl.device)
+    elif out.shape != (Do, Ho, Wo, cout) or out.dtype != torch.float32 or out.device != x_cl.device or not out.is_contiguous():
+        raise ValueError("conv3d_sbf: out must be a contiguous fp32 [Do,Ho,Wo,cout] tensor on the input's device")
     if skip is not None and skip.shape != out.shape:
         raise ValueError("conv3d_sbf: residual shape mismatch")
     if wsplit.dtype != torch.int16 or not wsplit.is_cuda or not wsplit.is_contiguous():
diff --git a/include/cds_mvsnet_hip.h b/include/cds_mvsnet_hip.h
--- a/include/cds_mvsnet_hip.h
+++ b/include/cds_mvsnet_hip.h
@@ -86,6 +86,7 @@
                        int Cin, int Cout, int D, int H, int W, int stride, int act, void* stream);
 int cds_conv3d_sf16_f32(const float* x, const void* weight_split, const float* bias, float* out, int Cin, int Cout, int D, int H, int W,
                         int stride, int act, const float* in_bound, float w_inv_scale, float* out_bound, void* stream);
+int cds_conv3d_zmg_plan(int Cin, int Cout, int D, int H, int W, int stride, int f16, int* workgroups, int* units_per_workgroup);
 
 
 int cds_deconv3d_sbf_f32(const float* x, const void* weight_split, const float* bias, const float* skip, float* out,
```
